# benlaktibyassine/DocQA-MS-Clinical-Document-QA-Assistant-LLM-Microservices-

Measured on AMD Instinct MI355X. Metric: e2e_qa_queries_per_sec, higher is better.
Workload: dtype bf16; 1 GPU; model=llama3-8b generator + minilm-l6 embedder + flat-L2 kNN (k=3), global_batch=256, seq_len=2048, parallelism=dp1, index_vectors=2647, kv_blocks=26451

## Files before the change

### docqa-ms-clinical-document-qa-assistant-llm-microservices-_amd/csrc/bindings.cpp

```cpp
#include <torch/library.h>
#include <algorithm>
#include <tuple>
#include <ATen/ATen.h>
#include <c10/hip/HIPStream.h>
#include <c10/core/DeviceGuard.h>

#include "docqa_kernels.h"

namespace {

hipStream_t stream() { return c10::hip::getCurrentHIPStream().stream(); }

#define CHECK_GPU(t) TORCH_CHECK((t).is_cuda(), #t " must be a GPU tensor")
#define CHECK_BF16(t) TORCH_CHECK((t).scalar_type() == at::kBFloat16, #t " must be bfloat16")
#define CHECK_I32(t) TORCH_CHECK((t).scalar_type() == at::kInt, #t " must be int32")
#define CHECK_CONTIG(t) TORCH_CHECK((t).is_contiguous(), #t " must be contiguous")
#define CHECK_ALIGN16(t) \
  TORCH_CHECK((reinterpret_cast<uintptr_t>((t).data_ptr()) & 15u) == 0, \
              #t " must be 16-byte aligned (storage offset a multiple of 16 bytes)")
static bool kernel_debug() {
  static const bool on = [] {
    const char* e = getenv("DOCQA_KERNEL_DEBUG");
    return e && atoi(e) != 0;
  }();
// ... 579 lines not shown
                                      pml.data_ptr<float>(), order_ptr(order, B), stream()),
           "paged_decode_cascade");
  return out;
}

at::Tensor paged_decode_cascade_grouped(const at::Tensor& q, at::Tensor k_cache, at::Tensor v_cache,
                                        const at::Tensor& block_tables, const at::Tensor& context_lens,
                                        int64_t Hq, double scale, const at::Tensor& prefix_table,
                                        const at::Tensor& prefix_len, int64_t nchunk, const at::Tensor& groups) {
  CHECK_GPU(q); CHECK_BF16(q); CHECK_BF16(k_cache); CHECK_BF16(v_cache);
  CHECK_I32(block_tables); CHECK_I32(context_lens); CHECK_CONTIG(block_tables);
  CHECK_I32(prefix_table); CHECK_I32(prefix_len); CHECK_CONTIG(prefix_table);
  CHECK_I32(groups); CHECK_CONTIG(groups);
  TORCH_CHECK(q.stride(-1) == 1, "q rows must be contiguous");
  const int B = q.size(0);
  const int Hkv = k_cache.size(1), BS = k_cache.size(2), D = k_cache.size(3);
  TORCH_CHECK(D == 128 && BS == 64 && Hq == 4 * Hkv, "grouped decode: head_dim 128, 64-token blocks, GQA 4");
  TORCH_CHECK(block_tables.size(1) <= 256, "grouped decode: block table <= 256 wide (rows <= 64 blocks: the caller)");
  TORCH_CHECK(context_lens.numel() == B && block_tables.size(0) >= B, "grouped decode: B rows");
  TORCH_CHECK(groups.numel() % 4 == 0 && groups.numel() >= 4, "groups: [ngroups, 4]");
  TORCH_CHECK(prefix_table.numel() >= 1 && prefix_len.numel() == 1, "cascade decode: prefix table / length");
  c10::DeviceGuard g(q.device());
  auto out = at::empty({B, Hq * D}, q.options());
  auto f32 = q.options().dtype(at::kFloat);
  auto pacc = at::empty({nchunk, B, Hq, D}, f32);
  auto pml = at::empty({nchunk, B, Hq, 2}, f32);
  CHECK_RC(docqa_paged_decode_cascade_grouped(q.data_ptr(), q.stride(0), k_cache.data_ptr(), v_cache.data_ptr(),
                                              block_tables.data_ptr<int>(), block_tables.size(1),
                                              context_lens.data_ptr<int>(), out.data_ptr(), Hq * D, B, Hq, Hkv,
                                              BS, (float)scale, prefix_table.data_ptr<int>(),
                                              prefix_len.data_ptr<int>(), (int)nchunk, pacc.data_ptr<float>(),
                                              pml.data_ptr<float>(), groups.data_ptr<int>(),
                                              (int)(groups.numel() / 4), stream()),
           "paged_decode_cascade_grouped");
  return out;
}

at::Tensor paged_decode_grouped_fused(const at::Tensor& P, const at::Tensor& positions, const at::Tensor& cos_sin,
                                      const at::Tensor& slot_mapping, at::Tensor k_cache, at::Tensor v_cache,
                                      const at::Tensor& block_tables, const at::Tensor& context_lens, int64_t Hq,
                                      double scale, const at::Tensor& prefix_table, const at::Tensor& prefix_len,
                                      int64_t nchunk, const at::Tensor& plan, const c10::optional<at::Tensor>& tick) {
  CHECK_GPU(P); CHECK_CONTIG(P); CHECK_BF16(k_cache); CHECK_BF16(v_cache);
  CHECK_I32(positions); CHECK_I32(slot_mapping); CHECK_I32(block_tables); CHECK_I32(context_lens);
  CHECK_CONTIG(block_tables); CHECK_I32(prefix_table); CHECK_I32(prefix_len); CHECK_I32(plan); CHECK_CONTIG(plan);
  TORCH_CHECK(P.scalar_type() == at::kFloat && P.dim() == 3, "fused grouped decode: slabs fp32 [S, B, width]");
  TORCH_CHECK(cos_sin.scalar_type() == at::kFloat, "cos_sin must be fp32");
  const int B = P.size(1);
  const int Hkv = k_cache.size(1), BS = k_cache.size(2), D = k_cache.size(3);
  TORCH_CHECK(D == 128 && BS == 64 && Hq == 4 * Hkv && P.size(2) == (Hq + 2 * Hkv) * D,
              "fused grouped decode: head_dim 128, 64-token blocks, GQA 4, packed QKV width");
  TORCH_CHECK(block_tables.size(1) <= 256 && context_lens.numel() == B && block_tables.size(0) >= B &&
              positions.numel() >= B && slot_mapping.numel() >= B, "fused grouped decode: B rows, block table <= 256 wide");
  TORCH_CHECK(plan.dim() == 3 && plan.size(0) == 2 && plan.size(2) == 8, "fused grouped decode: split plan [2, cap, 8]");
  const int cap = plan.size(1);
  c10::DeviceGuard g(P.device());
  auto out = at::empty({B, Hq * D}, P.options().dtype(at::kBFloat16));
  auto f32 = P.options();
  auto ws_acc = at::empty({cap, Hkv, 16, D}, f32);
  auto ws_ml = at::empty({cap, Hkv, 16, 2}, f32);
  int* tick_ptr = nullptr;
  if (tick && tick->defined()) {
    CHECK_GPU((*tick)); CHECK_I32((*tick));
    TORCH_CHECK(tick->numel() >= (int64_t)cap * Hkv, "fused grouped decode: tick needs cap * Hkv entries");
    tick_ptr = tick->data_ptr<int>();
  }
  const int* pp = plan.data_ptr<int>();
  CHECK_RC(docqa_paged_decode_cascade_split(nullptr, 0, k_cache.data_ptr(), v_cache.data_ptr(),
                                            block_tables.data_ptr<int>(), block_tables.size(1),
                                            context_lens.data_ptr<int>(), out.data_ptr(), Hq * D, B, Hq, Hkv, BS,
                                            (float)scale, prefix_table.data_ptr<int>(), prefix_len.data_ptr<int>(),
                                            (int)nchunk, nullptr, nullptr, pp, pp + 8 * cap, cap,
                                            ws_acc.data_ptr<float>(), ws_ml.data_ptr<float>(), 0, stream(), tick_ptr, 1,
                                            P.data_ptr<float>(), P.size(0), positions.data_ptr<int>(),
                                            cos_sin.data_ptr<float>(), slot_mapping.data_ptr<int>()),
           "paged_decode_grouped_fused");
  return out;
}

at::Tensor paged_decode_cascade_split(const at::Tensor& q, at::Tensor k_cache, at::Tensor v_cache,
                                      const at::Tensor& block_tables, const at::Tensor& context_lens,
                                      int64_t Hq, double scale, const at::Tensor& prefix_table,
                                      const at::Tensor& prefix_len, int64_t nchunk, const at::Tensor& plan,
                                      bool defer, const c10::optional<at::Tensor>& tick, bool inline_prefix) {
  CHECK_GPU(q); CHECK_BF16(q);
  TORCH_CHECK(k_cache.dim() == 4, "k_cache: [num_blocks, Hkv, BS, D]");
  const bool f8 = kv_fp8(k_cache, v_cache, k_cache.size(1), k_cache.size(3));
  TORCH_CHECK(!f8 || (inline_prefix && !defer && plan.dim() == 3 && plan.size(0) == 2),
              "split decode (fp8 cache): a [2, cap, 8] plan from block 0 (inline_prefix), not deferred");
  CHECK_I32(block_tables); CHECK_I32(context_lens); CHECK_CONTIG(block_tables);
  CHECK_I32(prefix_table); CHECK_I32(prefix_len); CHECK_CONTIG(prefix_table);
  CHECK_I32(plan); CHECK_CONTIG(plan);
  TORCH_CHECK(q.stride(-1) == 1, "q rows must be contiguous");
  const int B = q.size(0);
  const int Hkv = k_cache.size(1), BS = k_cache.size(2), D = k_cache.size(3);
  TORCH_CHECK(D == 128 && BS == 64 && Hq == 4 * Hkv, "split decode: head_dim 128, 64-token blocks, GQA 4");
  TORCH_CHECK(block_tables.size(1) <= 256, "split decode: block table <= 256 wide (rows <= 64 blocks: the caller)");
  TORCH_CHECK(k_cache.size(0) < (1 << 20), "split decode: < 2^20 KV blocks (packed tile lists)");
  TORCH_CHECK(context_lens.numel() == B && block_tables.size(0) >= B, "split decode: B rows");
  TORCH_CHECK(plan.dim() == 3 && plan.size(0) >= 2 && plan.size(0) <= 3 && plan.size(2) == 8 && plan.size(1) >= 1,
              "plan: [2, cap, 8] (split) or [3, cap, 8] (persistent bins)");
  TORCH_CHECK(prefix_table.numel() >= 1 && prefix_len.numel() == 1, "cascade decode: prefix table / length");
  const int cap = plan.size(1);
  c10::DeviceGuard g(q.device());
  auto out = at::empty({B, Hq * D}, q.options());
  auto f32 = q.options().dtype(at::kFloat);
  auto pacc = f8 ? at::Tensor() : at::empty({nchunk, B, Hq, D}, f32);
  auto pml = f8 ? at::Tensor() : at::empty({nchunk, B, Hq, 2}, f32);
  auto ws_acc = at::empty({cap, Hkv, 16, D}, f32);
  auto ws_ml = at::empty({cap, Hkv, 16, 2}, f32);
  const int* pp = plan.data_ptr<int>();
  int* tick_ptr = nullptr;
  if (tick && tick->defined()) {
    CHECK_GPU((*tick)); CHECK_I32((*tick));
    TORCH_CHECK(tick->numel() >= (int64_t)cap * Hkv, "split decode: tick needs cap * Hkv entries");
    tick_ptr = tick->data_ptr<int>();
  }
  if (f8) {
    TORCH_CHECK(q.dim() == 2 && q.size(1) >= Hq * D && q.stride(0) % 8 == 0, "split decode (fp8 cache): q rows");
    CHECK_ALIGN16(q);
    CHECK_RC(docqa_paged_decode_group_wave8(q.data_ptr(), q.stride(0), k_cache.data_ptr(), v_cache.data_ptr(),
                                            block_tables.data_ptr<int>(), block_tables.size(1),
                                            context_lens.data_ptr<int>(), out.data_ptr(), Hq * D, B, Hq, Hkv, BS,
                                            (float)scale, pp, pp + 8 * cap, cap, ws_acc.data_ptr<float>(),
                                            ws_ml.data_ptr<float>(), stream(), tick_ptr),
             "paged_decode_cascade_split (fp8 cache)");
    return out;
  }
  if (plan.size(0) == 3) {
    CHECK_RC(docqa_paged_decode_cascade_persist(q.data_ptr(), q.stride(0), k_cache.data_ptr(), v_cache.data_ptr(),
                                                block_tables.data_ptr<int>(), block_tables.size(1),
                                                context_lens.data_ptr<int>(), out.data_ptr(), Hq * D, B, Hq, Hkv,
                                                BS, (float)scale, prefix_table.data_ptr<int>(),
                                                prefix_len.data_ptr<int>(), (int)nchunk, pacc.data_ptr<float>(),
                                                pml.data_ptr<float>(), pp, pp + 8 * cap, pp + 16 * cap, cap,
                                                ws_acc.data_ptr<float>(), ws_ml.data_ptr<float>(), stream()),
             "paged_decode_cascade_persist");
    return out;
  }
  CHECK_RC(docqa_paged_decode_cascade_split(q.data_ptr(), q.stride(0), k_cache.data_ptr(), v_cache.data_ptr(),
                                            block_tables.data_ptr<int>(), block_tables.size(1),
                                            context_lens.data_ptr<int>(), out.data_ptr(), Hq * D, B, Hq, Hkv,
                                            BS, (float)scale, prefix_table.data_ptr<int>(),
                                            prefix_len.data_ptr<int>(), (int)nchunk, pacc.data_ptr<float>(),
                                            pml.data_ptr<float>(), pp, pp + 8 * cap, cap, ws_acc.data_ptr<float>(),
                                            ws_ml.data_ptr<float>(), defer ? 1 : 0, stream(), tick_ptr,
                                            inline_prefix ? 1 : 0),
           "paged_decode_cascade_split");
  return out;
}

at::Tensor paged_decode_cascade_rope(at::Tensor qkv, const at::Tensor& positions, const at::Tensor& cos_sin,
                                     const at::Tensor& slot_mapping, at::Tensor k_cache, at::Tensor v_cache,
                                     const at::Tensor& block_tables, const at::Tensor& context_lens,
                                     int64_t Hq, int64_t max_context, double scale,
                                     const at::Tensor& prefix_table, const at::Tensor& prefix_len,
                                     int64_t nchunk, const c10::optional<at::Tensor>& order) {
  CHECK_GPU(qkv); CHECK_BF16(qkv); CHECK_BF16(k_cache); CHECK_BF16(v_cache);
  CHECK_I32(positions); CHECK_I32(slot_mapping); CHECK_I32(block_tables); CHECK_I32(context_lens);
  CHECK_CONTIG(block_tables); CHECK_I32(prefix_table); CHECK_I32(prefix_len); CHECK_CONTIG(prefix_table);
  TORCH_CHECK(qkv.dim() == 2 && qkv.stride(1) == 1, "qkv must be [B, width] with unit stride");
  TORCH_CHECK(cos_sin.scalar_type() == at::kFloat, "cos_sin must be fp32");
  const int B = qkv.size(0);
  const int Hkv = k_cache.size(1), BS = k_cache.size(2), D = k_cache.size(3);
  TORCH_CHECK(D == 128 && BS == 64 && Hq == 4 * Hkv, "cascade decode: head_dim 128, 64-token blocks, GQA 4");
  TORCH_CHECK(qkv.size(1) >= (Hq + 2 * Hkv) * D, "qkv rows narrower than the packed QKV width");
  TORCH_CHECK(positions.numel() == B && slot_mapping.numel() == B && context_lens.numel() == B,
              "positions / slot_mapping / context_lens must have B entries");
  TORCH_CHECK(block_tables.size(1) <= 256, "cascade decode: <= 256 blocks per sequence");
  TORCH_CHECK(prefix_table.numel() >= 1 && prefix_len.numel() == 1, "cascade decode: prefix table / length");
  const int max_parts = docqa_decode_splits(B, Hkv, max_context);
  c10::DeviceGuard g(qkv.device());
  auto out = at::empty({B, Hq * D}, qkv.options());
  auto f32 = qkv.options().dtype(at::kFloat);
  auto tmp_out = at::empty({B, Hq, max_parts, D}, f32);
  auto tmp_ml = at::empty({B, Hq, max_parts, 2}, f32);
  auto pacc = at::empty({nchunk, B, Hq, D}, f32);
  auto pml = at::empty({nchunk, B, Hq, 2}, f32);
  CHECK_RC(docqa_paged_decode_cascade_rope(qkv.data_ptr(), qkv.stride(0), positions.data_ptr<int>(),
                                           cos_sin.data_ptr<float>(), slot_mapping.data_ptr<int>(),
                                           k_cache.data_ptr(), v_cache.data_ptr(), block_tables.data_ptr<int>(),
                                           block_tables.size(1), context_lens.data_ptr<int>(), out.data_ptr(),
                                           Hq * D, tmp_out.data_ptr<float>(), tmp_ml.data_ptr<float>(), B, Hq,
                                           Hkv, BS, max_parts, (float)scale, prefix_table.data_ptr<int>(),
                                           prefix_len.data_ptr<int>(), (int)nchunk, pacc.data_ptr<float>(),
                                           pml.data_ptr<float>(), order_ptr(order, B), stream()),
           "paged_decode_cascade_rope");
  return out;
}

at::Tensor paged_decode_fused(const at::Tensor& P, const at::Tensor& positions, const at::Tensor& cos_sin,
                              const at::Tensor& slot_mapping, at::Tensor k_cache, at::Tensor v_cache,
                              const at::Tensor& block_tables, const at::Tensor& context_lens,
                              int64_t Hq, int64_t max_context, double scale,
                              const c10::optional<at::Tensor>& order, const c10::optional<at::Tensor>& tick) {
  CHECK_GPU(P); CHECK_CONTIG(P); CHECK_BF16(k_cache); CHECK_BF16(v_cache);
  CHECK_I32(positions); CHECK_I32(slot_mapping); CHECK_I32(block_tables); CHECK_I32(context_lens);
  CHECK_CONTIG(block_tables);
  TORCH_CHECK(P.scalar_type() == at::kFloat && P.dim() == 3, "partials must be fp32 [S, B, width]");
  TORCH_CHECK(cos_sin.scalar_type() == at::kFloat, "cos_sin must be fp32");
  const int B = P.size(1);
  const int Hkv = k_cache.size(1), BS = k_cache.size(2), D = k_cache.size(3);
  TORCH_CHECK(D == 128 && P.size(2) == (Hq + 2 * Hkv) * D, "fused decode: head_dim 128, packed QKV width");
  const int max_parts = docqa_decode_splits(B, Hkv, max_context);
  c10::DeviceGuard g(P.device());
  auto out = at::empty({B, Hq * D}, P.options().dtype(at::kBFloat16));
  auto tmp_out = at::empty({B, Hq, max_parts, D}, P.options());
  auto tmp_ml = at::empty({B, Hq, max_parts, 2}, P.options());
  int* tick_ptr = nullptr;
  if (tick && tick->defined()) {
    CHECK_GPU((*tick)); CHECK_I32((*tick));
    TORCH_CHECK(tick->numel() >= (int64_t)B * Hkv, "paged_decode_fused: tick needs B * Hkv entries");
    tick_ptr = tick->data_ptr<int>();
  }
  CHECK_RC(docqa_paged_decode_fused(P.data_ptr<float>(), P.size(0), positions.data_ptr<int>(),
                                    cos_sin.data_ptr<float>(), slot_mapping.data_ptr<int>(),
                                    k_cache.data_ptr(), v_cache.data_ptr(), block_tables.data_ptr<int>(),
                                    block_tables.size(1), context_lens.data_ptr<int>(), out.data_ptr(),
                                    Hq * D, tmp_out.data_ptr<float>(), tmp_ml.data_ptr<float>(), B, Hq,
                                    Hkv, BS, max_parts, (float)scale, order_ptr(order, B), stream(), tick_ptr),
           "paged_decode_fused");
  return out;
}

at::Tensor flash_prefill(const at::Tensor& qkv, const at::Tensor& cu_seqlens, int64_t max_len,
                         int64_t Hq, int64_t Hkv, int64_t D, double scale, bool causal) {
  CHECK_GPU(qkv); CHECK_BF16(qkv); CHECK_I32(cu_seqlens);
  TORCH_CHECK(qkv.stride(-1) == 1 && qkv.size(-1) == (Hq + 2 * Hkv) * D, "qkv layout mismatch");
  const int T = qkv.numel() / qkv.size(-1);
  const int B = cu_seqlens.numel() - 1;
  c10::DeviceGuard g(qkv.device());
  auto out = at::empty({T, Hq * D}, qkv.options());
// ... 908 lines not shown
  m.def("sample(Tensor logits, Tensor inv_temp, Tensor top_k, Tensor top_p, Tensor u) -> Tensor");
  m.def("penalty_window() -> int", &penalty_window);
  m.def("apply_penalties(Tensor(a!) logits, Tensor hist, Tensor hist_n, Tensor last_n, Tensor rep_pen, "
        "Tensor pres_pen, Tensor freq_pen, Tensor? valid=None) -> ()");
  m.def("penalized_argmax(Tensor(a!) logits, int n_valid, Tensor hist, Tensor hist_n, Tensor last_n, "
        "Tensor rep_pen, Tensor pres_pen, Tensor freq_pen, Tensor? valid=None) -> Tensor");
  m.def("top_logprobs_max() -> int", &top_logprobs_max);
  m.def("token_logprobs(Tensor logits, int n_valid, Tensor chosen, Tensor top_n, Tensor(a!) lp, "
        "Tensor(b!) top_ids, Tensor(c!) top_lp) -> ()");
  m.def("decode_advance_hist(Tensor nxt, Tensor(a!) out, Tensor(b!) tokens, Tensor(c!) positions, "
        "Tensor(d!) context_lens, Tensor valid, Tensor(e!) hist, Tensor(f!) hist_n) -> ()");
  m.def("paged_decode(Tensor q, Tensor k_cache, Tensor v_cache, Tensor block_tables, "
        "Tensor context_lens, int Hq, int max_context, float scale, Tensor? order=None) -> Tensor");
  m.def("flash_prefill(Tensor qkv, Tensor cu_seqlens, int max_len, int Hq, int Hkv, int D, "
        "float scale, bool causal) -> Tensor");
  m.def("knn(Tensor xb, Tensor xb_norms, Tensor xq, int k, bool inner_product, int id_offset) "
        "-> (Tensor, Tensor)");
  m.def("pool_l2(Tensor h, Tensor cu_seqlens, bool mean, bool normalize) -> Tensor");
  m.def("coarse_probes(Tensor xq, Tensor cent, Tensor cnorm, int nprobe) -> Tensor");
  m.def("fp32_gemm_nt(Tensor x, Tensor w) -> Tensor");
  m.def("ivfpq_search(Tensor xq, Tensor centroids, Tensor pq, Tensor codes, Tensor ids, "
        "Tensor list_off, Tensor probes, int k) -> (Tensor, Tensor)");
  m.def("ivfpq_search_pt(Tensor xq, Tensor centroids, Tensor pq, Tensor codes, Tensor norms, Tensor ids, "
        "Tensor list_off, Tensor probes, int k, int pc) -> (Tensor, Tensor)");
  m.def("refine_flat(Tensor xb, Tensor xq, Tensor cand, int k, bool ip) -> (Tensor, Tensor)");
  m.def("pq_encode(Tensor x, Tensor centroids, Tensor assign, Tensor pq) -> Tensor");
  m.def("gemm(Tensor a, Tensor w, Tensor? bias, Tensor? residual, int epi) -> Tensor");
  m.def("flash_prefill_paged(Tensor qkv, Tensor cu_seqlens, int max_len, int Hq, int Hkv, int D, "
        "float scale, Tensor k_cache, Tensor v_cache, Tensor block_tables, Tensor ctx_start) -> Tensor");
  m.def("dgemm(Tensor x, Tensor w, int splits) -> Tensor");
  m.def("dgemm_partial(Tensor x, Tensor w, int splits, int tile_rows=64) -> Tensor");
  m.def("embed_rmsnorm(Tensor ids, Tensor table, Tensor w, float eps) -> (Tensor, Tensor)");
  m.def("dgemm_partial_xn(Tensor Pin, Tensor res_in, Tensor(a!) res_out, Tensor gamma, float eps, Tensor w, "
        "int splits) -> Tensor");
  m.def("dgemm_glu_xn(Tensor Pin, Tensor res_in, Tensor(a!) res_out, Tensor gamma, float eps, Tensor w) -> Tensor");
  m.def("gemv(Tensor x, Tensor w, int splits=1, int rows=16, bool glu=False) -> Tensor");
  m.def("gemv_xn(Tensor Pin, Tensor res_in, Tensor(a!) res_out, Tensor gamma, float eps, Tensor w, int splits=1, int rows=16, bool glu=False) -> Tensor");
  m.def("dgemm_add_rmsnorm(Tensor x, Tensor w, int splits, Tensor(a!) residual, Tensor gamma, float eps, "
        "Tensor(t!) tick) -> Tensor");
  m.def("dgemm_glu(Tensor x, Tensor w) -> Tensor");
  m.def("mgemm(Tensor x, Tensor w, int splits, int cfg=0) -> Tensor");
  m.def("mgemm_slab16(Tensor x, Tensor w, int splits, int cfg=0) -> Tensor");
  m.def("mgemm_glu(Tensor x, Tensor w, int cfg=0) -> Tensor");
  m.def("mgemm_tile_n(int cfg) -> int", &mgemm_tile_n);
  m.def("mgemm_argmax(Tensor x, Tensor w, int n_valid, int cfg=0) -> Tensor");
  m.def("dgemm_argmax_val(Tensor x, Tensor w, int n_valid) -> (Tensor, Tensor)");
  m.def("gemv_argmax_val(Tensor x, Tensor w, int n_valid) -> (Tensor, Tensor)");
  m.def("gemv4(Tensor x, Tensor q, Tensor e, int splits=1, int rows=16, int lb=32, int kw=1, bool glu=False) -> Tensor");
  m.def("gemv4_xn(Tensor Pin, Tensor res_in, Tensor(a!) res_out, Tensor gamma, float eps, Tensor q, Tensor e, "
        "int splits=1, int rows=16, int lb=32, int kw=1, bool glu=False) -> Tensor");
  m.def("gemv4_argmax_val(Tensor x, Tensor q, Tensor e, int n_valid, int rows=16, int lb=32, int kw=1) "
        "-> (Tensor, Tensor)");
  m.def("gemv8(Tensor x, Tensor q, Tensor scale, int splits=1, int rows=16, int lb=8, bool glu=False) -> Tensor");
  m.def("gemv8_xn(Tensor Pin, Tensor res_in, Tensor(a!) res_out, Tensor gamma, float eps, Tensor q, Tensor scale, "
        "int splits=1, int rows=16, int lb=8, bool glu=False) -> Tensor");
  m.def("gemv8_argmax_val(Tensor x, Tensor q, Tensor scale, int n_valid, int rows=16, int lb=8) -> (Tensor, Tensor)");
  m.def("dgemm8_partial(Tensor x, Tensor q, Tensor scale, int splits, int tile_rows=64) -> Tensor");
  m.def("dgemm8_glu(Tensor x, Tensor q, Tensor scale) -> Tensor");
  m.def("dgemm8_argmax_val(Tensor x, Tensor q, Tensor scale, int n_valid) -> (Tensor, Tensor)");
  m.def("dgemm8w_partial(Tensor x, Tensor q, Tensor scale, int splits, int tile_rows=128) -> Tensor");
  m.def("dgemm8w_glu(Tensor x, Tensor q, Tensor scale) -> Tensor");
  m.def("dgemm8w_argmax_val(Tensor x, Tensor q, Tensor scale, int n_valid) -> (Tensor, Tensor)");
  m.def("dgemm4_partial(Tensor x, Tensor q, Tensor e, int splits, int tile_rows=64) -> Tensor");
  m.def("dgemm4_glu(Tensor x, Tensor q, Tensor e) -> Tensor");
  m.def("dgemm4_argmax_val(Tensor x, Tensor q, Tensor e, int n_valid) -> (Tensor, Tensor)");
  m.def("pgemm(Tensor x, Tensor w, int epi=0) -> Tensor");
  m.def("pgemm_partial(Tensor x, Tensor w, int splits) -> Tensor");
  m.def("mgemm_argmax_val(Tensor x, Tensor w, int n_valid, int cfg=0) -> (Tensor, Tensor)");
  m.def("pgemm_ok(int M, int N, int K) -> bool", &pgemm_ok);
  m.def("mgemm_ld(Tensor x, Tensor w, int splits, int cfg, bool glu) -> Tensor");
  m.def("group_persist_bins(int cap, int Hkv) -> int", &group_persist_bins);
  m.def("set_decode_trace(Tensor? buf) -> ()", &set_decode_trace);
  m.def("set_group_wave(int on) -> int", &set_group_wave);
  m.def("paged_decode_cascade(Tensor q, Tensor k_cache, Tensor v_cache, Tensor block_tables, "
        "Tensor context_lens, int Hq, int max_context, float scale, Tensor prefix_table, Tensor prefix_len, "
        "int nchunk, Tensor? order=None) -> Tensor");
  m.def("paged_decode_cascade_grouped(Tensor q, Tensor k_cache, Tensor v_cache, Tensor block_tables, "
        "Tensor context_lens, int Hq, float scale, Tensor prefix_table, Tensor prefix_len, int nchunk, "
        "Tensor groups) -> Tensor");
  m.def("kv_copy_rows(Tensor caches, Tensor tab, int num_blocks, int Hkv, int BS, int D) -> ()");
  m.def("kv_copy_rows8(Tensor caches, Tensor tab, int num_blocks, int Hkv, int BS, int D) -> ()");
  m.def("paged_decode_cascade_split(Tensor q, Tensor k_cache, Tensor v_cache, Tensor block_tables, "
        "Tensor context_lens, int Hq, float scale, Tensor prefix_table, Tensor prefix_len, int nchunk, "
        "Tensor plan, bool defer=False, Tensor(t!)? tick=None, bool inline_prefix=False) -> Tensor");
  m.def("paged_decode_grouped_fused(Tensor P, Tensor positions, Tensor cos_sin, Tensor slot_mapping, "
        "Tensor(a!) k_cache, Tensor(b!) v_cache, Tensor block_tables, Tensor context_lens, int Hq, float scale, "
        "Tensor prefix_table, Tensor prefix_len, int nchunk, Tensor plan, Tensor(t!)? tick=None) -> Tensor");
  m.def("paged_decode_cascade_rope(Tensor(a!) qkv, Tensor positions, Tensor cos_sin, Tensor slot_mapping, "
        "Tensor(b!) k_cache, Tensor(c!) v_cache, Tensor block_tables, Tensor context_lens, int Hq, "
        "int max_context, float scale, Tensor prefix_table, Tensor prefix_len, int nchunk, "
        "Tensor? order=None) -> Tensor");
  m.def("paged_decode_fused(Tensor P, Tensor positions, Tensor cos_sin, Tensor slot_mapping, "
        "Tensor(a!) k_cache, Tensor(b!) v_cache, Tensor block_tables, Tensor context_lens, int Hq, "
        "int max_context, float scale, Tensor? order=None, Tensor(t!)? tick=None) -> Tensor");
  m.def("ar_run(Tensor x, bool slabs, Tensor(r!)? residual, Tensor? w, float eps, int rank, int[] regions, "
        "int max_elems, int mode, Tensor(a!) ctr, Tensor(b!) err, int timeout_us=500000) -> Tensor");
  m.def("ar_region_bytes(int max_elems) -> int", &ar_region_bytes);
  m.def("ar_alloc(int bytes) -> int", &ar_alloc);
  m.def("ar_free(int ptr) -> ()", &ar_free);
  m.def("ar_ipc_handle(int ptr) -> Tensor", &ar_ipc_handle);
  m.def("ar_ipc_open(Tensor handle) -> int", &ar_ipc_open);
  m.def("ar_ipc_close(int ptr) -> ()", &ar_ipc_close);
  m.def("add_rmsnorm_splitk(Tensor P, Tensor(a!) residual, Tensor w, float eps) -> Tensor");
  m.def("rope_cache_splitk(Tensor P, Tensor positions, Tensor cos_sin, Tensor? slot_mapping, "
        "Tensor(b!) k_cache, Tensor(c!) v_cache, int Hq, int Hkv, int D) -> Tensor");
}

TORCH_LIBRARY_IMPL(docqa, CUDA, m) {
  m.impl("rmsnorm", &rmsnorm);
  m.impl("add_rmsnorm", &add_rmsnorm);
  m.impl("layernorm", &layernorm);
  m.impl("rope_cache", &rope_cache);
  m.impl("silu_mul", &silu_mul);
  m.impl("silu_mul_splitk", &silu_mul_splitk);
  m.impl("bias_act", &bias_act);
  m.impl("embedding", &embedding);
  m.impl("bert_embed_ln", &bert_embed_ln);
  m.impl("argmax", &argmax);
  m.impl("token_cls_argmax", &token_cls_argmax);
  m.impl("decode_slots", &decode_slots);
  m.impl("decode_advance", &decode_advance);
  m.impl("sample", &sample);
  m.impl("apply_penalties", &apply_penalties);
  m.impl("penalized_argmax", &penalized_argmax);
  m.impl("token_logprobs", &token_logprobs);
  m.impl("decode_advance_hist", &decode_advance_hist);
  m.impl("paged_decode", &paged_decode);
  m.impl("flash_prefill", &flash_prefill);
  m.impl("knn", &knn);
  m.impl("pool_l2", &pool_l2);
  m.impl("ivfpq_search", &ivfpq_search);
  m.impl("ivfpq_search_pt", &ivfpq_search_pt);
  m.impl("refine_flat", &refine_flat);
  m.impl("pq_encode", &pq_encode);
  m.impl("gemm", &gemm);
  m.impl("flash_prefill_paged", &flash_prefill_paged);
  m.impl("dgemm", &dgemm);
  m.impl("dgemm_partial", &dgemm_partial);
  m.impl("embed_rmsnorm", &embed_rmsnorm);
  m.impl("dgemm_partial_xn", &dgemm_partial_xn);
  m.impl("dgemm_glu_xn", &dgemm_glu_xn);
  m.impl("gemv", &gemv);
  m.impl("gemv_xn", &gemv_xn);
  m.impl("dgemm_add_rmsnorm", &dgemm_add_rmsnorm);
  m.impl("dgemm_glu", &dgemm_glu);
  m.impl("mgemm", &mgemm);
  m.impl("mgemm_slab16", &mgemm_slab16);
  m.impl("mgemm_glu", &mgemm_glu);
  m.impl("mgemm_argmax", &mgemm_argmax);
  m.impl("pgemm", &pgemm);
  m.impl("mgemm_ld", &mgemm_ld);
  m.impl("pgemm_partial", &pgemm_partial);
  m.impl("mgemm_argmax_val", &mgemm_argmax_val);
  m.impl("coarse_probes", &coarse_probes);
  m.impl("fp32_gemm_nt", &fp32_gemm_nt);
  m.impl("dgemm_argmax_val", &dgemm_argmax_val);
  m.impl("gemv_argmax_val", &gemv_argmax_val);
  m.impl("gemv4", &gemv4);
  m.impl("gemv4_xn", &gemv4_xn);
  m.impl("gemv4_argmax_val", &gemv4_argmax_val);
  m.impl("gemv8", &gemv8);
  m.impl("gemv8_xn", &gemv8_xn);
  m.impl("gemv8_argmax_val", &gemv8_argmax_val);
  m.impl("dgemm8_partial", &dgemm8_partial);
  m.impl("dgemm8_glu", &dgemm8_glu);
  m.impl("dgemm8_argmax_val", &dgemm8_argmax_val);
  m.impl("dgemm8w_partial", &dgemm8w_partial);
  m.impl("dgemm8w_glu", &dgemm8w_glu);
  m.impl("dgemm8w_argmax_val", &dgemm8w_argmax_val);
  m.impl("dgemm4_partial", &dgemm4_partial);
  m.impl("dgemm4_glu", &dgemm4_glu);
  m.impl("dgemm4_argmax_val", &dgemm4_argmax_val);
  m.impl("paged_decode_fused", &paged_decode_fused);
  m.impl("paged_decode_cascade", &paged_decode_cascade);
  m.impl("paged_decode_cascade_rope", &paged_decode_cascade_rope);
  m.impl("paged_decode_cascade_grouped", &paged_decode_cascade_grouped);
  m.impl("paged_decode_cascade_split", &paged_decode_cascade_split);
  m.impl("paged_decode_grouped_fused", &paged_decode_grouped_fused);
  m.impl("kv_copy_rows", &kv_copy_rows);
  m.impl("kv_copy_rows8", &kv_copy_rows8);
  m.impl("ar_run", &ar_run);
  m.impl("add_rmsnorm_splitk", &add_rmsnorm_splitk);
  m.impl("rope_cache_splitk", &rope_cache_splitk);
}
```

### docqa-ms-clinical-document-qa-assistant-llm-microservices-_amd/csrc/include/docqa_kernels.h

```cpp
#pragma once
#include <hip/hip_runtime.h>
#include <stdint.h>

int docqa_rmsnorm(const void* x, const void* w, void* out, int rows, int H, float eps,
                  hipStream_t s);
int docqa_add_rmsnorm(const void* x, void* residual, const void* w, void* out, int rows, int H,
                      float eps, hipStream_t s);
int docqa_layernorm(const void* x, const void* residual, const void* g, const void* b, void* out,
                    int rows, int H, float eps, hipStream_t s);

int docqa_kv_copy_rows(const uint64_t* caches, int ntensors, const int* tab, int n, int nblocks, int Hkv, int BS,
                       int D, hipStream_t s);
int docqa_rope_cache(void* qkv, const int* positions, const float* cos_sin,
                     const int* slot_mapping, void* k_cache, void* v_cache, int T, int Hq,
                     int Hkv, int D, int row_stride, int BS, hipStream_t s);

int docqa_kv_copy_rows8(const uint64_t* caches, int ntensors, const int* tab, int n, int nblocks, int Hkv, int BS,
                        int D, hipStream_t s);
int docqa_rope_cache8(void* qkv, const int* positions, const float* cos_sin, const int* slot_mapping,
                      void* k_cache, void* v_cache, int T, int Hq, int Hkv, int D, int row_stride, int BS,
                      hipStream_t s);
int docqa_rope_cache_splitk8(const void* P, int slab16, int S, void* qkv_out, const int* positions,
                             const float* cos_sin, const int* slot_mapping, void* k_cache, void* v_cache, int T,
                             int Hq, int Hkv, int D, int row_stride, int BS, hipStream_t s);
int docqa_flash_prefill_paged8(const void* qkv, int row_stride, const int* cu_seqlens, void* out,
                               int o_stride, int B, int max_len, int Hq, int Hkv, int head_dim,
                               float scale, const void* k_cache, const void* v_cache,
                               const int* block_tables, int maxb, const int* ctx_start, int BS,
                               hipStream_t s);
int docqa_paged_decode8(const void* q, int q_stride, const void* k_cache, const void* v_cache,
                        const int* block_tables, int maxb, const int* context_lens, void* out,
                        int out_stride, float* tmp_out, float* tmp_ml, int B, int Hq, int Hkv,
                        int D, int BS, int max_parts, float scale, hipStream_t s);
int docqa_paged_decode_group_wave8(const void* q, int q_stride, const void* k_cache, const void* v_cache,
                                   const int* block_tables, int maxb, const int* context_lens, void* out,
                                   int out_stride, int B, int Hq, int Hkv, int BS, float scale, const int* items,
                                   const int* merges, int cap, float* ws_acc, float* ws_ml, hipStream_t s,
                                   int* tick);

int docqa_silu_mul(const void* gu, void* out, int T, int I, int interleaved, hipStream_t s);
int docqa_silu_mul_splitk16(const void* P, void* out, int S, int T, int I, hipStream_t s);
int docqa_silu_mul_splitk(const float* P, void* out, int S, int T, int I, hipStream_t s);
int docqa_bias_act(const void* x, const void* bias, const void* res, void* out, int T, int N,
                   int gelu, hipStream_t s);

int docqa_embedding(const int* ids, const void* table, void* out, int T, int H, int V, hipStream_t s);
int docqa_decode_slots(const int* block_tables, int maxb, const int* positions, const int* valid,
                       int* slots, int B, int BS, hipStream_t s);
int docqa_decode_advance(const int64_t* nxt, int64_t* out, int* tokens, int* positions,
                         int* context_lens, const int* valid, int B, hipStream_t s);
int docqa_bert_embed_ln(const int* ids, const int* pos, const int* tt, const void* wte,
                        const void* wpe, const void* wtt, const void* g, const void* b, void* out,
                        int T, int H, float eps, hipStream_t s);
int docqa_argmax(const void* logits, int rows, int V, int ld, int is_bf16, float* ws_v, int* ws_i,
                 int splits, int64_t* out, hipStream_t s);
int docqa_token_cls_argmax(const void* h, int ldh, const void* w, const void* bias, int n_rows,
                           int n_valid, int T, int H, int64_t* out, hipStream_t s);
int docqa_sample(const float* logits, int rows, int V, int ld, const float* inv_temp,
                 const int* top_k, const float* top_p, const float* u, int64_t* out,
                 hipStream_t s);

int docqa_penalty_window();
int docqa_apply_penalties(float* logits, int rows, int V, int ld, const int* hist, int W,
                          const int* hist_n, const int* last_n, const float* rep, const float* pres,
                          const float* freq, const int* valid, hipStream_t s);
int docqa_penalized_argmax(void* logits, int rows, int V, int ld, int n_valid, int is_bf16,
                           const int* hist, int W, const int* hist_n, const int* last_n,
                           const float* rep, const float* pres, const float* freq, const int* valid,
                           float* ws_v, int* ws_i, int splits, float* pen_v, int* pen_i,
                           int64_t* out, hipStream_t s);
int docqa_decode_advance_hist(const int64_t* nxt, int64_t* out, int* tokens, int* positions,
                              int* context_lens, const int* valid, int* hist, int W, int* hist_n,
                              int B, hipStream_t s);

int docqa_top_logprobs_max();
int docqa_token_logprobs_splits(int rows, int V, int* chunk_out);
int docqa_token_logprobs(const void* logits, int rows, int n_valid, int ld, int is_bf16, const int64_t* chosen,
                         const int* top_n, float* pm, float* ps, float* ptv, int* pti, float* lp, int* top_ids,
                         float* top_lp, hipStream_t s);

int docqa_paged_decode(const void* q, int q_stride, const void* k_cache, const void* v_cache,
                       const int* block_tables, int maxb, const int* context_lens, void* out,
                       int out_stride, float* tmp_out, float* tmp_ml, int B, int Hq, int Hkv,
                       int D, int BS, int max_parts, float scale, const int* order, hipStream_t s);
int docqa_decode_splits(int B, int Hkv, int max_context);
int docqa_paged_decode_cascade(const void* q, int q_stride, void* k_cache, void* v_cache,
                               const int* block_tables, int maxb, const int* context_lens, void* out,
                               int out_stride, float* tmp_out, float* tmp_ml, int B, int Hq, int Hkv,
                               int BS, int max_parts, float scale, const int* prefix_table,
                               const int* plen, int nchunk, float* pacc, float* pml, const int* order,
                               hipStream_t s);
int docqa_paged_decode_cascade_grouped(const void* q, int q_stride, void* k_cache, void* v_cache,
                                       const int* block_tables, int maxb, const int* context_lens,
                                       void* out, int out_stride, int B, int Hq, int Hkv, int BS,
                                       float scale, const int* prefix_table, const int* plen, int nchunk,
                                       float* pacc, float* pml, const int* groups, int ngroups,
                                       hipStream_t s);
int docqa_paged_decode_cascade_split(const void* q, int q_stride, void* k_cache, void* v_cache,
                                     const int* block_tables, int maxb, const int* context_lens,
                                     void* out, int out_stride, int B, int Hq, int Hkv, int BS,
                                     float scale, const int* prefix_table, const int* plen, int nchunk,
                                     float* pacc, float* pml, const int* items, const int* merges, int cap,
                                     float* ws_acc, float* ws_ml, int defer,
                                     hipStream_t s, int* tick = nullptr, int inline_prefix = 0,
                                     const float* fP = nullptr, int fS = 0, const int* positions = nullptr,
                                     const float* cos_sin = nullptr, const int* slot_mapping = nullptr);
int docqa_paged_decode_cascade_persist(const void* q, int q_stride, void* k_cache, void* v_cache,
                                       const int* block_tables, int maxb, const int* context_lens,
                                       void* out, int out_stride, int B, int Hq, int Hkv, int BS,
                                       float scale, const int* prefix_table, const int* plen, int nchunk,
                                       float* pacc, float* pml, const int* items, const int* merges,
                                       const int* bins, int cap, float* ws_acc, float* ws_ml, hipStream_t s);
int docqa_group_persist_bins(int cap, int Hkv);
int docqa_set_decode_trace(long long* buf);
int docqa_set_group_wave(int on);
int docqa_paged_decode_cascade_rope(void* qkv, int q_stride, const int* positions,
                                    const float* cos_sin, const int* slot_mapping, void* k_cache,
                                    void* v_cache, const int* block_tables, int maxb,
                                    const int* context_lens, void* out, int out_stride,
                                    float* tmp_out, float* tmp_ml, int B, int Hq, int Hkv, int BS,
                                    int max_parts, float scale, const int* prefix_table,
                                    const int* plen, int nchunk, float* pacc, float* pml,
                                    const int* order, hipStream_t s);

int docqa_flash_prefill(const void* qkv, int row_stride, const int* cu_seqlens, void* out,
                        int o_stride, int B, int max_len, int Hq, int Hkv, int head_dim,
                        float scale, int causal, hipStream_t s);

int docqa_flash_prefill_paged(const void* qkv, int row_stride, const int* cu_seqlens, void* out,
                              int o_stride, int B, int max_len, int Hq, int Hkv, int head_dim,
                              float scale, const void* k_cache, const void* v_cache,
                              const int* block_tables, int maxb, const int* ctx_start, int BS,
                              hipStream_t s);

int docqa_dgemm_partial(const void* X, const void* W, float* P, int M, int N, int K, int S,
                        int tile_rows, hipStream_t s);
int docqa_add_rmsnorm_splitk(const float* P, int S, void* residual, const void* w, void* out,
                             int rows, int H, float eps, hipStream_t s);
int docqa_rope_cache_splitk(const float* P, int S, void* qkv_out, const int* positions,
                            const float* cos_sin, const int* slot_mapping, void* k_cache,
                            void* v_cache, int T, int Hq, int Hkv, int D, int row_stride, int BS,
                            hipStream_t s);
int docqa_add_rmsnorm_splitk16(const void* P, int S, void* residual, const void* w, void* out,
                               int rows, int H, float eps, hipStream_t s);
int docqa_rope_cache_splitk16(const void* P, int S, void* qkv_out, const int* positions,
                              const float* cos_sin, const int* slot_mapping, void* k_cache,
                              void* v_cache, int T, int Hq, int Hkv, int D, int row_stride, int BS,
                              hipStream_t s);
size_t docqa_ar_region_bytes(size_t max_elems);
int docqa_ar_alloc(size_t bytes, void** ptr);
int docqa_ar_free(void* ptr);
int docqa_ar_ipc_handle(void* ptr, void* handle_out);
int docqa_ar_ipc_open(const void* handle, void** ptr);
int docqa_ar_ipc_close(void* ptr);
int docqa_ar_run(const void* in, int S, void* out, void* residual, const void* w, float eps, int M, int H,
                 int rank, int nranks, void* const* regions, size_t max_elems, int mode, unsigned* ctr,
                 unsigned* err, long long timeout_us, hipStream_t s);
int docqa_paged_decode_fused(const float* P, int S, const int* positions, const float* cos_sin,
                             const int* slot_mapping, void* k_cache, void* v_cache,
                             const int* block_tables, int maxb, const int* context_lens, void* out,
                             int out_stride, float* tmp_out, float* tmp_ml, int B, int Hq, int Hkv,
                             int BS, int max_parts, float scale, const int* order, hipStream_t s,
                             int* tick = nullptr);
int docqa_dgemm_splits(int N, int K);
int docqa_dgemm_glu(const void* X, const void* W, void* Y, int M, int N, int K, hipStream_t s);
int docqa_dgemm_add_rmsnorm(const void* X, const void* W, float* P, int M, int N, int K, int S, void* residual,
                            const void* gamma, void* out, float eps, int* tick, hipStream_t s);
int docqa_dgemm_partial_xn(const float* Pin, int Sin, const void* res_in, void* res_out, const void* gamma,
                           float eps, const void* W, float* P, int N, int K, int S, hipStream_t s);
int docqa_dgemm_glu_xn(const float* Pin, int Sin, const void* res_in, void* res_out, const void* gamma, float eps,
                       const void* W, void* Y, int N, int K, hipStream_t s);
int docqa_gemv(const void* X, const void* W, void* Y, float* P, int N, int K, int S, int R, int epi,
               const float* Pin, int Sin, const void* res_in, void* res_out, const void* gamma, float eps,
               hipStream_t s);
int docqa_gemv8(const void* X, const void* Wq, const float* scale, void* Y, float* P, int N, int K, int S, int R,
                int LB, int epi, const float* Pin, int Sin, const void* res_in, void* res_out, const void* gamma,
                float eps, hipStream_t s);
int docqa_gemv8_argmax(const void* X, const void* Wq, const float* scale, int64_t* out, float* outv, float* ws_v,
                       int* ws_i, int N, int K, int R, int LB, int n_valid, hipStream_t s);
int docqa_gemv4(const void* X, const void* Wq, const void* E, void* Y, float* P, int N, int K, int S, int R, int LB,
                int KW, int epi, const float* Pin, int Sin, const void* res_in, void* res_out, const void* gamma,
                float eps, hipStream_t s);
int docqa_gemv4_argmax(const void* X, const void* Wq, const void* E, int64_t* out, float* outv, float* ws_v,
                       int* ws_i, int N, int K, int R, int LB, int KW, int n_valid, hipStream_t s);
int docqa_dgemm8_partial(const void* X, const void* Wq, const float* scale, float* P, int M, int N, int K, int S,
                         int tile_rows, hipStream_t s);
int docqa_dgemm8_glu(const void* X, const void* Wq, const float* scale, void* Y, int M, int N, int K, hipStream_t s);
int docqa_dgemm8_argmax(const void* X, const void* Wq, const float* scale, int64_t* out, float* outv, float* ws_v,
                        int* ws_i, int M, int N, int K, int n_valid, hipStream_t s);
// ... 58 lines not shown
```

### docqa-ms-clinical-document-qa-assistant-llm-microservices-_amd/csrc/kernels/attn_decode.hip

```cpp
#include "docqa_common.h"
#include "docqa_asm.h"
#include "docqa_cascade.h"
#include "docqa_norm_row.h"
#include <float.h>
#include <stdlib.h>
#include <type_traits>

using namespace docqa;

constexpr int kMinChunk = 64;
typedef __attribute__((address_space(3))) i16x4 lds_i16x4;

static int hpw_knob() {
  static const int v = [] {
    const char* e = getenv("DOCQA_DECODE_HPW");
    return e ? atoi(e) : 1;
  }();
  return v;
}

static int mfma_nsr() {
  static const int v = [] {
    const char* e = getenv("DOCQA_DECODE_NSR");
    return e ? atoi(e) : 4;
// ... 1131 lines not shown
    const bool mine = (e.y & cbit) != 0;
    const int base = (e.y >> 8) * 64 + ((e.y >> 4) & 1) * TT;
    const uint16_t* kt = ring + (jt % NSR) * 2 * TILE;
    const uint16_t* vt = kt + TILE;
    f32x4 x[2];
#pragma unroll
    for (int c = 0; c < 2; ++c) {
      x[c] = f32x4{0.f, 0.f, 0.f, 0.f};
      const int t = 16 * c + hl;
#pragma unroll
      for (int ks = 0; ks < 4; ++ks) {
        const bf16x8 a = *reinterpret_cast<const bf16x8*>(kt + t * D + (((4 * ks + lg) ^ (t & 15)) << 3));
        x[c] = __builtin_amdgcn_mfma_f32_16x16x32_bf16(a, qf[ks], x[c], 0, 0, 0);
      }
    }
    float mx = -FLT_MAX;
#pragma unroll
    for (int c = 0; c < 2; ++c)
#pragma unroll
      for (int r = 0; r < 4; ++r) {
        const int tok = base + 16 * c + 4 * lg + r;
        const float v = (mine && tok < cL) ? x[c][r] * qs : -FLT_MAX;
        x[c][r] = v;
        mx = fmaxf(mx, v);
      }
    mx = fmaxf(mx, __shfl_xor(mx, 16, 64));
    mx = fmaxf(mx, __shfl_xor(mx, 32, 64));
    const float m_new = fmaxf(m, mx);
    const float alpha = m_new == -FLT_MAX ? 1.f : exp2f(m - m_new);
    float ps = 0.f;
#pragma unroll
    for (int c = 0; c < 2; ++c)
#pragma unroll
      for (int r = 0; r < 4; ++r) {
        const float p = x[c][r] == -FLT_MAX ? 0.f : exp2f(x[c][r] - m_new);
        x[c][r] = p;
        ps += p;
      }
    ps += __shfl_xor(ps, 16, 64);
    ps += __shfl_xor(ps, 32, 64);
    l = l * alpha + ps;
    m = m_new;
#pragma unroll
    for (int dd = 0; dd < 2; ++dd) acc[dd] *= alpha;
#pragma unroll
    for (int c = 0; c < 2; ++c) {
      i16x4 pb;
#pragma unroll
      for (int r = 0; r < 4; ++r) pb[r] = (short)f2bf(x[c][r]);
      const int row = 16 * c + 4 * lg + (hl >> 2), pp = hl & 3;
#pragma unroll
      for (int dd = 0; dd < 2; ++dd) {
        const int ch = 2 * (2 * wave + dd) + (pp >> 1);
        const uint16_t* va = vt + row * D + ((ch ^ vswz(row)) << 3) + 4 * (pp & 1);
        const i16x4 a = __builtin_amdgcn_ds_read_tr16_b64_v4i16((lds_i16x4*)va);
        acc[dd] = __builtin_amdgcn_mfma_f32_16x16x16bf16_1k(a, pb, acc[dd], 0, 0, 0);
      }
    }
  }
  wait_vmcnt<0>();
  if (trace && tid == 0) tr3 = wall_clock64();

  trace_out();
  group_item_finish<SPLIT>(m, l, acc, part, crow, cL, hl, lg, wave, tid, gp, merges, tick, ws_acc, ws_ml, ci,
                           context_lens, B, Hkv, out, out_stride, kvh, P);
}

typedef unsigned int u32x2_t __attribute__((ext_vector_type(2)));
__device__ __forceinline__ float rows4_max(float x) {
  const u32x2_t a = __builtin_amdgcn_permlane16_swap(__float_as_uint(x), __float_as_uint(x), false, false);
  const float h0 = __uint_as_float(a.x), h1 = __uint_as_float(a.y);
  const float y = h0 > h1 ? h0 : h1;
  const u32x2_t b = __builtin_amdgcn_permlane32_swap(__float_as_uint(y), __float_as_uint(y), false, false);
  const float g0 = __uint_as_float(b.x), g1 = __uint_as_float(b.y);
  return g0 > g1 ? g0 : g1;
}
__device__ __forceinline__ float rows4_sum(float x) {
  const u32x2_t a = __builtin_amdgcn_permlane16_swap(__float_as_uint(x), __float_as_uint(x), false, false);
  const float y = __uint_as_float(a.x) + __uint_as_float(a.y);
  const u32x2_t b = __builtin_amdgcn_permlane32_swap(__float_as_uint(y), __float_as_uint(y), false, false);
  return __uint_as_float(b.x) + __uint_as_float(b.y);
}

template <int WAVES, int NSRW>
__global__ __launch_bounds__(64 * WAVES) void paged_decode_group_wave_kernel(
    const uint16_t* __restrict__ q, int q_stride, const uint16_t* __restrict__ k_cache,
    const uint16_t* __restrict__ v_cache, const int* __restrict__ block_tables, int maxb,
    const int* __restrict__ context_lens, int B, int Hkv, float scale,
    uint16_t* __restrict__ out, int out_stride, const int* __restrict__ groups, CascadeIn ci,
    float* __restrict__ ws_acc, float* __restrict__ ws_ml, const int* __restrict__ merges, int* __restrict__ tick) {
  constexpr int G = 4, R = 4, D = 128, TQ = 16, MAXT = kGroupMaxPos * 16;
  constexpr int TILE = TQ * D;
  constexpr int WSLOT = 2 * TILE;
  constexpr int NDT = 8 / WAVES;
  static_assert(WAVES * NSRW * WSLOT * 2 >= WAVES * 8 * 64 * 16 + WAVES * 16 * 2 * 4, "ring reused by the merge");
  __shared__ __attribute__((aligned(16))) uint16_t ring[WAVES * NSRW * WSLOT];
  __shared__ unsigned s_tl[MAXT];
  __shared__ int s_nt;

  const int kvh = blockIdx.x, grp = blockIdx.y;
  const int tid = threadIdx.x, lane = tid & 63;
  const int wave = __builtin_amdgcn_readfirstlane(tid >> 6);
  const int hl = lane & 15, lg = lane >> 4;
  long long* trace = g_group_trace;
  long long tr0 = 0, tr1 = 0, tr2 = 0, tr3 = 0;
  if (trace && tid == 0) tr0 = wall_clock64();
  const int P = ci.plen ? *ci.plen : 0;
  const int* gp = groups + 8 * grp;
  int rows[R], Ls[R];
#pragma unroll
  for (int r = 0; r < R; ++r) {
    const int row = gp[r];
    rows[r] = row >= 0 && row < B ? row : -1;
    Ls[r] = rows[r] >= 0 ? context_lens[rows[r]] : 0;
  }
  if (rows[0] < 0 && rows[1] < 0 && rows[2] < 0 && rows[3] < 0) return;
  const int lo = gp[4], hi = min(gp[5], maxb), part = gp[6];

  if (wave == 0) {
    const int pos = max(P >> 6, lo) + lane;
    int ids[R], nq[R], mk[R];
#pragma unroll
    for (int r = 0; r < R; ++r) ids[r] = rows[r] >= 0 && pos < hi ? block_tables[(size_t)rows[r] * maxb + pos] : -1;
    bool alive[R];
#pragma unroll
    for (int r = 0; r < R; ++r) {
      alive[r] = pos < hi && 64 * pos < Ls[r];
      ids[r] = alive[r] ? ids[r] : -1;
    }
    int cnt = 0;
#pragma unroll
    for (int r = 0; r < R; ++r) {
      bool first = alive[r];
#pragma unroll
      for (int r2 = 0; r2 < r; ++r2) first = first && !(alive[r2] && ids[r2] == ids[r]);
      int mask = 0, need = 0;
      if (first) {
#pragma unroll
        for (int r2 = 0; r2 < R; ++r2)
          if (alive[r2] && ids[r2] == ids[r]) {
            mask |= 1 << r2;
            need = max(need, min(4, (Ls[r2] - 64 * pos + TQ - 1) / TQ));
          }
      }
      nq[r] = need;
      mk[r] = mask;
      cnt += need;
    }
    int off = cnt;
#pragma unroll
    for (int o = 1; o < 64; o <<= 1) {
      const int v = __shfl_up(off, o, 64);
      if (lane >= o) off += v;
    }
    const int total = __shfl(off, 63, 64);
    off -= cnt;
#pragma unroll
    for (int r = 0; r < R; ++r)
      for (int h = 0; h < nq[r]; ++h) s_tl[off++] = ((unsigned)ids[r] << 12) | (pos << 6) | (h << 4) | mk[r];
    if (lane == 0) s_nt = total;
  }
  const int crow = rows[hl >> 2], cL = Ls[hl >> 2], cbit = 1 << (hl >> 2);
  bf16x8 qf[4];
  {
    const uint16_t* qp = q + (size_t)max(crow, 0) * q_stride + (size_t)(kvh * G + (hl & 3)) * D + lg * 8;
#pragma unroll
    for (int ks = 0; ks < 4; ++ks) {
      const uint4 v = crow >= 0 ? *reinterpret_cast<const uint4*>(qp + ks * 32) : make_uint4(0, 0, 0, 0);
      qf[ks] = __builtin_bit_cast(bf16x8, v);
    }
  }
  __syncthreads();
  const int nt = s_nt;
  if (trace && tid == 0) tr1 = wall_clock64();

  const float qs = scale * kLog2e;
  const uint32_t wbase = lds_u32(ring) + (uint32_t)(wave * NSRW * WSLOT * 2);
  const int prow = lane >> 4, pslot = lane & 15;
  const int mine_nt = nt > wave ? (nt - wave + WAVES - 1) / WAVES : 0;
  auto stage = [&](int i) {
    const unsigned e = s_tl[wave + WAVES * i];
    const size_t row0 = ((size_t)(e >> 12) * Hkv + kvh) * 64 + ((e >> 4) & 3) * TQ;
    const uint16_t* kp = k_cache + row0 * D;
    const uint16_t* vp = v_cache + row0 * D;
    const uint32_t dst = wbase + (uint32_t)((i % NSRW) * WSLOT * 2);
#pragma unroll
    for (int c = 0; c < 4; ++c) {
      const int t = 4 * c + prow;
      glds16<true>(kp + t * D + ((pslot ^ t) << 3), dst + c * 1024);
      glds16<true>(vp + t * D + ((pslot ^ vswz(t)) << 3), dst + TILE * 2 + c * 1024);
    }
  };
#pragma unroll
  for (int i = 0; i < NSRW - 1; ++i)
    if (i < mine_nt) stage(i);
  float m = -FLT_MAX, l = 0.f;
  f32x4 o8[8];
#pragma unroll
  for (int dt = 0; dt < 8; ++dt) o8[dt] = f32x4{0.f, 0.f, 0.f, 0.f};
  for (int i = 0; i < mine_nt; ++i) {
    if (i + NSRW - 1 < mine_nt) {
      stage(i + NSRW - 1);
      wait_vmcnt<8 * (NSRW - 1)>();
    } else {
      wait_vmcnt<0>();
    }
    if (trace && tid == 0 && i == 0) tr2 = wall_clock64();
    const unsigned e = s_tl[wave + WAVES * i];
    const bool mine = (e & cbit) != 0;
    const int base = ((e >> 6) & 63) * 64 + ((e >> 4) & 3) * TQ;
    const uint16_t* kt = ring + (wave * NSRW + i % NSRW) * WSLOT;
    const uint16_t* vt = kt + TILE;
    f32x4 x = f32x4{0.f, 0.f, 0.f, 0.f};
#pragma unroll
    for (int ks = 0; ks < 4; ++ks) {
      const bf16x8 a = *reinterpret_cast<const bf16x8*>(kt + hl * D + (((4 * ks + lg) ^ hl) << 3));
      x = __builtin_amdgcn_mfma_f32_16x16x32_bf16(a, qf[ks], x, 0, 0, 0);
    }
    float mx = -FLT_MAX;
#pragma unroll
    for (int r = 0; r < 4; ++r) {
      const int tok = base + 4 * lg + r;
      const float v = (mine && tok < cL) ? x[r] * qs : -FLT_MAX;
      x[r] = v;
      mx = fmaxf(mx, v);
    }
    mx = rows4_max(mx);
    const float m_new = fmaxf(m, mx);
    const float alpha = m_new == -FLT_MAX ? 1.f : __builtin_amdgcn_exp2f(m - m_new);
    float ps = 0.f;
#pragma unroll
    for (int r = 0; r < 4; ++r) {
      const float p = x[r] == -FLT_MAX ? 0.f : __builtin_amdgcn_exp2f(x[r] - m_new);
      x[r] = p;
      ps += p;
    }
    ps = rows4_sum(ps);
    l = l * alpha + ps;
    m = m_new;
    i16x4 pb;
#pragma unroll
    for (int r = 0; r < 4; ++r) pb[r] = (short)f2bf(x[r]);
    const int row = 4 * lg + (hl >> 2), pp = hl & 3;
#pragma unroll
    for (int dt = 0; dt < 8; ++dt) {
      o8[dt] *= alpha;
      const int ch = 2 * dt + (pp >> 1);
      const uint16_t* va = vt + row * D + ((ch ^ vswz(row)) << 3) + 4 * (pp & 1);
      const i16x4 a = __builtin_amdgcn_ds_read_tr16_b64_v4i16((lds_i16x4*)va);
      o8[dt] = __builtin_amdgcn_mfma_f32_16x16x16bf16_1k(a, pb, o8[dt], 0, 0, 0);
    }
  }
  if (trace && tid == 0) tr3 = wall_clock64();

  __syncthreads();
  f32x4* s_o = reinterpret_cast<f32x4*>(ring);
  float* s_ml = reinterpret_cast<float*>(ring) + WAVES * 8 * 64 * 4;
#pragma unroll
  for (int dt = 0; dt < 8; ++dt) s_o[(wave * 8 + dt) * 64 + lane] = o8[dt];
  if (lg == 0) {
    s_ml[(wave * 16 + hl) * 2] = m;
    s_ml[(wave * 16 + hl) * 2 + 1] = l;
  }
  __syncthreads();
  float mw[WAVES], lw[WAVES], M = -FLT_MAX;
#pragma unroll
  for (int u = 0; u < WAVES; ++u) {
    mw[u] = s_ml[(u * 16 + hl) * 2];
    lw[u] = s_ml[(u * 16 + hl) * 2 + 1];
    M = fmaxf(M, mw[u]);
  }
  f32x4 acc[NDT];
#pragma unroll
  for (int dd = 0; dd < NDT; ++dd) acc[dd] = f32x4{0.f, 0.f, 0.f, 0.f};
  float L = 0.f;
#pragma unroll
  for (int u = 0; u < WAVES; ++u) {
    const float f = mw[u] == -FLT_MAX ? 0.f : exp2f(mw[u] - M);
    L += f * lw[u];
#pragma unroll
    for (int dd = 0; dd < NDT; ++dd) acc[dd] += f * s_o[(u * 8 + NDT * wave + dd) * 64 + lane];
  }
  if (trace && tid == 0) {
    long long* t = trace + ((size_t)blockIdx.y * gridDim.x + blockIdx.x) * 8;
    t[0] = tr0; t[1] = tr1; t[2] = tr2; t[3] = tr3; t[4] = wall_clock64(); t[5] = nt;
    t[6] = __builtin_amdgcn_s_getreg((31 << 11) | 4);
    t[7] = __builtin_amdgcn_s_getreg(20 | (3 << 11)) & 15;
  }
  group_item_finish<true, NDT>(M, L, acc, part, crow, cL, hl, lg, wave, tid, gp, merges, tick, ws_acc, ws_ml, ci,
                          context_lens, B, Hkv, out, out_stride, kvh, P);
}

__device__ __forceinline__ i16x4 widen4_fp8(uint32_t c) {
  const bf16x2 a = __builtin_amdgcn_cvt_scalef32_pk_bf16_fp8(c, 1.0f, false);
  const bf16x2 b = __builtin_amdgcn_cvt_scalef32_pk_bf16_fp8(c, 1.0f, true);
  const uint2 u{__builtin_bit_cast(uint32_t, a), __builtin_bit_cast(uint32_t, b)};
  return __builtin_bit_cast(i16x4, u);
}

template <int NSRW>
__global__ __launch_bounds__(256) void paged_decode_group_wave8_kernel(
    const uint16_t* __restrict__ q, int q_stride, const uint8_t* __restrict__ k_cache,
    const uint8_t* __restrict__ v_cache, const int* __restrict__ block_tables, int maxb,
    const int* __restrict__ context_lens, int B, int Hkv, float scale,
    uint16_t* __restrict__ out, int out_stride, const int* __restrict__ groups, CascadeIn ci,
    float* __restrict__ ws_acc, float* __restrict__ ws_ml, const int* __restrict__ merges, int* __restrict__ tick) {
  constexpr int WAVES = 4, G = 4, R = 4, D = 128, TQ = 16, MAXT = kGroupMaxPos * 16;
  constexpr int TILE = TQ * D;
  constexpr int WSLOT = 2 * TILE;
  constexpr int NDT = 8 / WAVES;
  static_assert(WAVES * NSRW * WSLOT >= WAVES * 8 * 64 * 16 + WAVES * 16 * 2 * 4, "ring reused by the merge");
  __shared__ __attribute__((aligned(16))) uint8_t ring[WAVES * NSRW * WSLOT];
  __shared__ unsigned s_tl[MAXT];
  __shared__ int s_nt;

  const int kvh = blockIdx.x, grp = blockIdx.y;
  const int tid = threadIdx.x, lane = tid & 63;
  const int wave = __builtin_amdgcn_readfirstlane(tid >> 6);
  const int hl = lane & 15, lg = lane >> 4;
  const int P = ci.plen ? *ci.plen : 0;
  const int* gp = groups + 8 * grp;
  int rows[R], Ls[R];
#pragma unroll
  for (int r = 0; r < R; ++r) {
    const int row = gp[r];
    rows[r] = row >= 0 && row < B ? row : -1;
    Ls[r] = rows[r] >= 0 ? context_lens[rows[r]] : 0;
  }
  if (rows[0] < 0 && rows[1] < 0 && rows[2] < 0 && rows[3] < 0) return;
  const int lo = gp[4], hi = min(gp[5], maxb), part = gp[6];

  if (wave == 0) {
    const int pos = max(P >> 6, lo) + lane;
    int ids[R], nq[R], mk[R];
#pragma unroll
    for (int r = 0; r < R; ++r) ids[r] = rows[r] >= 0 && pos < hi ? block_tables[(size_t)rows[r] * maxb + pos] : -1;
    bool alive[R];
#pragma unroll
    for (int r = 0; r < R; ++r) {
      alive[r] = pos < hi && 64 * pos < Ls[r];
      ids[r] = alive[r] ? ids[r] : -1;
    }
    int cnt = 0;
#pragma unroll
    for (int r = 0; r < R; ++r) {
      bool first = alive[r];
#pragma unroll
      for (int r2 = 0; r2 < r; ++r2) first = first && !(alive[r2] && ids[r2] == ids[r]);
      int mask = 0, need = 0;
      if (first) {
#pragma unroll
        for (int r2 = 0; r2 < R; ++r2)
          if (alive[r2] && ids[r2] == ids[r]) {
            mask |= 1 << r2;
            need = max(need, min(4, (Ls[r2] - 64 * pos + TQ - 1) / TQ));
          }
      }
      nq[r] = need;
      mk[r] = mask;
      cnt += need;
    }
    int off = cnt;
#pragma unroll
    for (int o = 1; o < 64; o <<= 1) {
      const int v = __shfl_up(off, o, 64);
      if (lane >= o) off += v;
    }
    const int total = __shfl(off, 63, 64);
    off -= cnt;
#pragma unroll
    for (int r = 0; r < R; ++r)
      for (int h = 0; h < nq[r]; ++h) s_tl[off++] = ((unsigned)ids[r] << 12) | (pos << 6) | (h << 4) | mk[r];
    if (lane == 0) s_nt = total;
  }
  const int crow = rows[hl >> 2], cL = Ls[hl >> 2], cbit = 1 << (hl >> 2);
  bf16x8 qf[4];
  {
    const uint16_t* qp = q + (size_t)max(crow, 0) * q_stride + (size_t)(kvh * G + (hl & 3)) * D + lg * 8;
#pragma unroll
    for (int ks = 0; ks < 4; ++ks) {
      const uint4 v = crow >= 0 ? *reinterpret_cast<const uint4*>(qp + ks * 32) : make_uint4(0, 0, 0, 0);
      qf[ks] = __builtin_bit_cast(bf16x8, v);
    }
  }
  __syncthreads();
  const int nt = s_nt;

  const float qs = scale * kLog2e;
  const uint32_t wbase = lds_u32(ring) + (uint32_t)(wave * NSRW * WSLOT);
  const int prow = lane >> 3, pslot = lane & 7;
  const int mine_nt = nt > wave ? (nt - wave + WAVES - 1) / WAVES : 0;
  auto stage = [&](int i) {
    const unsigned e = s_tl[wave + WAVES * i];
    const size_t row0 = ((size_t)(e >> 12) * Hkv + kvh) * 64 + ((e >> 4) & 3) * TQ;
    const uint8_t* kp = k_cache + row0 * D;
    const uint8_t* vp = v_cache + row0 * D;
    const uint32_t dst = wbase + (uint32_t)((i % NSRW) * WSLOT);
#pragma unroll
    for (int c = 0; c < 2; ++c) {
      const int t = 8 * c + prow;
      glds16<true>(kp + t * D + ((pslot ^ ((t >> 1) & 7)) << 4), dst + c * 1024);
      glds16<true>(vp + (t ^ ((t >> 2) & 1)) * D + (pslot << 4), dst + TILE + c * 1024);
    }
  };
#pragma unroll
  for (int i = 0; i < NSRW - 1; ++i)
    if (i < mine_nt) stage(i);
  float m = -FLT_MAX, l = 0.f;
  f32x4 o8[8];
#pragma unroll
  for (int dt = 0; dt < 8; ++dt) o8[dt] = f32x4{0.f, 0.f, 0.f, 0.f};
  for (int i = 0; i < mine_nt; ++i) {
    if (i + NSRW - 1 < mine_nt) {
      stage(i + NSRW - 1);
      wait_vmcnt<4 * (NSRW - 1)>();
    } else {
      wait_vmcnt<0>();
    }
    const unsigned e = s_tl[wave + WAVES * i];
    const bool mine = (e & cbit) != 0;
    const int base = ((e >> 6) & 63) * 64 + ((e >> 4) & 3) * TQ;
    const uint8_t* kt = ring + (wave * NSRW + i % NSRW) * WSLOT;
    const uint8_t* vt = kt + TILE;
    f32x4 x = f32x4{0.f, 0.f, 0.f, 0.f};
#pragma unroll
    for (int ks = 0; ks < 4; ++ks) {
      const uint2 c = *reinterpret_cast<const uint2*>(kt + hl * D + (((2 * ks + (lg >> 1)) ^ ((hl >> 1) & 7)) << 4) +
                                                      (lg & 1) * 8);
      const bf16x8 a = __builtin_bit_cast(bf16x8, widen8_fp8(c));
      x = __builtin_amdgcn_mfma_f32_16x16x32_bf16(a, qf[ks], x, 0, 0, 0);
    }
    float mx = -FLT_MAX;
#pragma unroll
    for (int r = 0; r < 4; ++r) {
      const int tok = base + 4 * lg + r;
      const float v = (mine && tok < cL) ? x[r] * qs : -FLT_MAX;
      x[r] = v;
      mx = fmaxf(mx, v);
    }
    mx = rows4_max(mx);
    const float m_new = fmaxf(m, mx);
    const float alpha = m_new == -FLT_MAX ? 1.f : __builtin_amdgcn_exp2f(m - m_new);
    float ps = 0.f;
#pragma unroll
    for (int r = 0; r < 4; ++r) {
      const float p = x[r] == -FLT_MAX ? 0.f : __builtin_amdgcn_exp2f(x[r] - m_new);
      x[r] = p;
      ps += p;
    }
    ps = rows4_sum(ps);
    l = l * alpha + ps;
    m = m_new;
    i16x4 pb;
#pragma unroll
    for (int r = 0; r < 4; ++r) pb[r] = (short)f2bf(x[r]);
    uint2 w[4];
#pragma unroll
    for (int j = 0; j < 4; ++j) {
      const int t = 4 * lg + j;
      w[j] = *reinterpret_cast<const uint2*>(vt + (t ^ ((t >> 2) & 1)) * D + hl * 8);
    }
#pragma unroll
    for (int ih = 0; ih < 2; ++ih) {
      const uint32_t w0 = ih ? w[0].y : w[0].x, w1 = ih ? w[1].y : w[1].x;
      const uint32_t w2 = ih ? w[2].y : w[2].x, w3 = ih ? w[3].y : w[3].x;
      const uint32_t a01 = __builtin_amdgcn_perm(w1, w0, 0x05010400u), a23 = __builtin_amdgcn_perm(w3, w2, 0x05010400u);
      const uint32_t c01 = __builtin_amdgcn_perm(w1, w0, 0x07030602u), c23 = __builtin_amdgcn_perm(w3, w2, 0x07030602u);
      const uint32_t tr[4] = {__builtin_amdgcn_perm(a23, a01, 0x05040100u), __builtin_amdgcn_perm(a23, a01, 0x07060302u),
                              __builtin_amdgcn_perm(c23, c01, 0x05040100u), __builtin_amdgcn_perm(c23, c01, 0x07060302u)};
// ... 424 lines not shown
  const CascadeIn ci{pacc, pml, plen, nchunk, nullptr};
  static const int nsr = [] {
    const char* e = getenv("DOCQA_GROUP_NSR");
    return e && atoi(e) == 4 ? 4 : 3;
  }();
  if (nsr == 4)
    paged_decode_group_kernel<4><<<dim3(Hkv, ngroups), 256, 0, s>>>(
        (const uint16_t*)q, q_stride, (const uint16_t*)k_cache, (const uint16_t*)v_cache, block_tables, maxb,
        context_lens, B, Hkv, scale, (uint16_t*)out, out_stride, groups, ci);
  else
    paged_decode_group_kernel<3><<<dim3(Hkv, ngroups), 256, 0, s>>>(
        (const uint16_t*)q, q_stride, (const uint16_t*)k_cache, (const uint16_t*)v_cache, block_tables, maxb,
        context_lens, B, Hkv, scale, (uint16_t*)out, out_stride, groups, ci);
  DOCQA_CHECK_LAUNCH();
  return 0;
}

static int cascade_prefix_forked(const void* q, int q_stride, int B, int Hq, int Hkv, float scale, void* k_cache,
                                 void* v_cache, const int* prefix_table, const int* plen, int BS, int nchunk,
                                 float* pacc, float* pml, hipStream_t s, hipEvent_t* join) {
  static const bool fork = [] {
    const char* e = getenv("DOCQA_CASCADE_FORK");
    return !(e && atoi(e) == 0);
  }();
  *join = nullptr;
  hipStream_t side = s;
  hipEvent_t ev_fork = nullptr, ev_join = nullptr;
  if (fork) {
    static hipStream_t streams[64] = {};
    static hipEvent_t evs[64][2] = {};
    int dev = 0;
    if (hipGetDevice(&dev) == hipSuccess && dev >= 0 && dev < 64) {
      hipStreamCaptureStatus cs = hipStreamCaptureStatusNone;
      if (!streams[dev] && hipStreamIsCapturing(s, &cs) == hipSuccess && cs == hipStreamCaptureStatusNone) {
        if (hipStreamCreateWithFlags(&streams[dev], hipStreamNonBlocking) != hipSuccess ||
            hipEventCreateWithFlags(&evs[dev][0], hipEventDisableTiming) != hipSuccess ||
            hipEventCreateWithFlags(&evs[dev][1], hipEventDisableTiming) != hipSuccess)
          streams[dev] = nullptr;
      }
      if (streams[dev] && evs[dev][0] && evs[dev][1]) {
        side = streams[dev];
        ev_fork = evs[dev][0];
        ev_join = evs[dev][1];
      }
    }
  }
  if (side != s) {
    if (hipEventRecord(ev_fork, s) != hipSuccess || hipStreamWaitEvent(side, ev_fork, 0) != hipSuccess) return -3;
  }
  const int rc = docqa_cascade_prefix(q, q_stride, B, Hq, Hkv, scale, k_cache, v_cache, prefix_table, plen, BS,
                                      nchunk, pacc, pml, nullptr, nullptr, side);
  if (rc) return rc;
  if (side != s) {
    if (hipEventRecord(ev_join, side) != hipSuccess) return -3;
    *join = ev_join;
  }
  return 0;
}

static int g_group_wave = -1;
static bool group_wave_on() {
  if (g_group_wave < 0) {
    const char* e = getenv("DOCQA_GROUP_WAVE");
    const int v = e ? atoi(e) : 1;
    g_group_wave = v >= 0 && v <= 4 ? v : 0;
  }
  return g_group_wave > 0;
}

int docqa_set_group_wave(int v) {
  group_wave_on();
  const int was = g_group_wave;
  if (v >= 0) g_group_wave = v <= 4 ? v : 0;
  return was;
}

int docqa_paged_decode_cascade_split(const void* q, int q_stride, void* k_cache, void* v_cache,
                                     const int* block_tables, int maxb, const int* context_lens,
                                     void* out, int out_stride, int B, int Hq, int Hkv, int BS,
                                     float scale, const int* prefix_table, const int* plen, int nchunk,
                                     float* pacc, float* pml, const int* items, const int* merges, int cap,
                                     float* ws_acc, float* ws_ml, int defer, hipStream_t s, int* tick,
                                     int inline_prefix, const float* fP, int fS, const int* positions,
                                     const float* cos_sin, const int* slot_mapping) {
  if (B == 0) return 0;
  if (BS != 64 || maxb > kGroupMaxTable || Hq != 4 * Hkv || nchunk < 1 || nchunk > kCascadeMaxChunks || cap < 1)
    return -1;
  if (inline_prefix && defer) return -1;
  hipEvent_t ev_join = nullptr;
  if (!inline_prefix) {
    const int rc = defer ? cascade_prefix_forked(q, q_stride, B, Hq, Hkv, scale, k_cache, v_cache, prefix_table,
                                                 plen, BS, nchunk, pacc, pml, s, &ev_join)
                         : docqa_cascade_prefix(q, q_stride, B, Hq, Hkv, scale, k_cache, v_cache, prefix_table, plen,
                                                BS, nchunk, pacc, pml, nullptr, nullptr, s);
    if (rc) return rc;
  }
  const CascadeIn ci{pacc, pml, inline_prefix ? nullptr : plen, nchunk, nullptr};
  static const int nsr = [] {
    const char* e = getenv("DOCQA_GROUP_NSR");
    return e && atoi(e) == 4 ? 4 : 3;
  }();
  int* tk = (tick && !defer) ? tick : nullptr;
  if (fP) {
    if (!inline_prefix || defer || fS < 1 || !positions || !cos_sin || !slot_mapping) return -1;
    const FusedQKV fz{fP, fS, positions, cos_sin, slot_mapping, Hq};
    paged_decode_group_kernel<3, true, true><<<dim3(Hkv, cap), 256, 0, s>>>(
        nullptr, 0, (const uint16_t*)k_cache, (const uint16_t*)v_cache, block_tables, maxb, context_lens, B, Hkv,
        scale, (uint16_t*)out, out_stride, items, ci, ws_acc, ws_ml, merges, tk, fz);
    DOCQA_CHECK_LAUNCH();
    if (tk) return 0;
  } else if (group_wave_on()) {
#define DOCQA_WAVE_LAUNCH(W_, N_)                                                                                 \
  paged_decode_group_wave_kernel<W_, N_><<<dim3(Hkv, cap), 64 * W_, 0, s>>>(                                     \
      (const uint16_t*)q, q_stride, (const uint16_t*)k_cache, (const uint16_t*)v_cache, block_tables, maxb,       \
      context_lens, B, Hkv, scale, (uint16_t*)out, out_stride, items, ci, ws_acc, ws_ml, merges, tk)
    switch (g_group_wave) {
      case 2: DOCQA_WAVE_LAUNCH(2, 3); break;
      case 3: DOCQA_WAVE_LAUNCH(2, 4); break;
      case 4: DOCQA_WAVE_LAUNCH(1, 4); break;
      default: DOCQA_WAVE_LAUNCH(4, 2); break;
    }
#undef DOCQA_WAVE_LAUNCH
  } else if (nsr == 4)
    paged_decode_group_kernel<4, true><<<dim3(Hkv, cap), 256, 0, s>>>(
        (const uint16_t*)q, q_stride, (const uint16_t*)k_cache, (const uint16_t*)v_cache, block_tables, maxb,
        context_lens, B, Hkv, scale, (uint16_t*)out, out_stride, items, ci, ws_acc, ws_ml, merges, tk);
  else
    paged_decode_group_kernel<3, true><<<dim3(Hkv, cap), 256, 0, s>>>(
        (const uint16_t*)q, q_stride, (const uint16_t*)k_cache, (const uint16_t*)v_cache, block_tables, maxb,
        context_lens, B, Hkv, scale, (uint16_t*)out, out_stride, items, ci, ws_acc, ws_ml, merges, tk);
  DOCQA_CHECK_LAUNCH();
  if (tk) return 0;
  if (ev_join && hipStreamWaitEvent(s, ev_join, 0) != hipSuccess) return -3;
  group_split_merge_kernel<<<dim3(Hkv, defer ? cap : (cap + 1) / 2), 256, 0, s>>>(merges, ws_acc, ws_ml, context_lens, B, Hkv,
                                                          (uint16_t*)out, out_stride, ci);
  DOCQA_CHECK_LAUNCH();
  return 0;
}

int docqa_paged_decode_group_wave8(const void* q, int q_stride, const void* k_cache, const void* v_cache,
                                   const int* block_tables, int maxb, const int* context_lens, void* out,
                                   int out_stride, int B, int Hq, int Hkv, int BS, float scale, const int* items,
                                   const int* merges, int cap, float* ws_acc, float* ws_ml, hipStream_t s,
                                   int* tick) {
  if (B == 0) return 0;
  if (BS != 64 || maxb > kGroupMaxTable || Hq != 4 * Hkv || cap < 1) return -1;
  const CascadeIn ci{nullptr, nullptr, nullptr, 1, nullptr};
  paged_decode_group_wave8_kernel<4><<<dim3(Hkv, cap), 256, 0, s>>>(
      (const uint16_t*)q, q_stride, (const uint8_t*)k_cache, (const uint8_t*)v_cache, block_tables, maxb,
      context_lens, B, Hkv, scale, (uint16_t*)out, out_stride, items, ci, ws_acc, ws_ml, merges, tick);
  DOCQA_CHECK_LAUNCH();
  if (tick) return 0;
  group_split_merge_kernel<<<dim3(Hkv, (cap + 1) / 2), 256, 0, s>>>(merges, ws_acc, ws_ml, context_lens, B, Hkv,
                                                                   (uint16_t*)out, out_stride, ci);
  DOCQA_CHECK_LAUNCH();
  return 0;
}

int docqa_paged_decode_cascade_persist(const void* q, int q_stride, void* k_cache, void* v_cache,
                                       const int* block_tables, int maxb, const int* context_lens,
                                       void* out, int out_stride, int B, int Hq, int Hkv, int BS,
                                       float scale, const int* prefix_table, const int* plen, int nchunk,
                                       float* pacc, float* pml, const int* items, const int* merges,
                                       const int* bins, int cap, float* ws_acc, float* ws_ml, hipStream_t s) {
  if (B == 0) return 0;
  if (BS != 64 || maxb > kGroupMaxTable || Hq != 4 * Hkv || nchunk < 1 || nchunk > kCascadeMaxChunks || cap < 1)
    return -1;
  hipEvent_t ev_join = nullptr;
  const int rc = cascade_prefix_forked(q, q_stride, B, Hq, Hkv, scale, k_cache, v_cache, prefix_table, plen, BS,
                                       nchunk, pacc, pml, s, &ev_join);
  if (rc) return rc;
  const CascadeIn ci{pacc, pml, plen, nchunk, nullptr};
  const int nb = group_persist_bins(cap, Hkv);
  paged_decode_group_persist_kernel<3><<<dim3(Hkv, nb), 256, 0, s>>>(
      (const uint16_t*)q, q_stride, (const uint16_t*)k_cache, (const uint16_t*)v_cache, block_tables, maxb,
      context_lens, B, Hkv, scale, items, bins, ci, ws_acc, ws_ml);
  DOCQA_CHECK_LAUNCH();
  if (ev_join && hipStreamWaitEvent(s, ev_join, 0) != hipSuccess) return -3;
  group_split_merge_kernel<<<dim3(Hkv, cap), 256, 0, s>>>(merges, ws_acc, ws_ml, context_lens, B, Hkv,
                                                          (uint16_t*)out, out_stride, ci);
  DOCQA_CHECK_LAUNCH();
  return 0;
}

int docqa_group_persist_bins(int cap, int Hkv) { return group_persist_bins(cap, Hkv); }

int docqa_set_decode_trace(long long* buf) {
  return hipMemcpyToSymbol(HIP_SYMBOL(g_group_trace), &buf, sizeof(buf)) == hipSuccess ? 0 : -1;
}

template <int D>
__global__ __launch_bounds__(D) void paged_decode_reduce(const float* __restrict__ tmp_out,
                                                         const float* __restrict__ tmp_ml,
                                                         const int* __restrict__ context_lens,
                                                         uint16_t* __restrict__ out,
                                                         int out_stride, int Hq, int max_parts,
                                                         CascadeIn ci = CascadeIn{}) {
  const int h = blockIdx.x, b = blockIdx.y, d = threadIdx.x;
  const int P = ci.plen ? *ci.plen : 0;
  const int L = context_lens[b] - P;
  if (L <= 0) {
    out[(size_t)b * out_stride + (size_t)h * D + d] = 0;
    return;
  }
  const int chunk = split_chunk(L, max_parts);
  const int np = min(max_parts, (L + chunk - 1) / chunk);
  const int nc = ci.plen ? cascade_parts(P, ci.nchunk) : 0;
  const size_t base = ((size_t)b * Hq + h) * max_parts;
  const size_t B = gridDim.y;
  float M = -FLT_MAX;
  for (int p = 0; p < np; ++p) M = fmaxf(M, tmp_ml[(base + p) * 2]);
  for (int c = 0; c < nc; ++c) M = fmaxf(M, ci.ml[((c * B + b) * Hq + h) * 2]);
  float num = 0.f, den = 0.f;
  for (int p = 0; p < np; ++p) {
    const float w = exp2f(tmp_ml[(base + p) * 2] - M);
    num += w * tmp_out[(base + p) * D + d];
    den += w * tmp_ml[(base + p) * 2 + 1];
  }
  for (int c = 0; c < nc; ++c) {
    const size_t r = (c * B + b) * Hq + h;
    const float pm = ci.ml[r * 2];
    const float w = (pm == -FLT_MAX) ? 0.f : exp2f(pm - M);
    num += w * ci.acc[r * D + d];
    den += w * ci.ml[r * 2 + 1];
  }
  out[(size_t)b * out_stride + (size_t)h * D + d] = f2bf(den > 0.f ? num / den : 0.f);
}

int docqa_paged_decode(const void* q, int q_stride, const void* k_cache, const void* v_cache,
                       const int* block_tables, int maxb, const int* context_lens, void* out,
                       int out_stride, float* tmp_out, float* tmp_ml, int B, int Hq, int Hkv,
                       int D, int BS, int max_parts, float scale, const int* order, hipStream_t s) {
  if (B == 0) return 0;
  if (D != 128 || (BS & (BS - 1)) != 0 || Hq % Hkv != 0) return -1;
  CascadeIn oi{};
  oi.order = order;
  int log2BS = 0;
  while ((1 << log2BS) < BS) ++log2BS;
  const int G = Hq / Hkv;
  dim3 grid(Hkv, B, max_parts);
  const bool direct = max_parts == 1;
  static const int u_env = [] {
    const char* e = getenv("DOCQA_DECODE_U");
    return e ? atoi(e) : 0;
  }();
#define DEC_K(GG, UU, DIR)                                                                    \
  paged_decode_kernel<GG, 128, UU, DIR><<<grid, 256, 0, s>>>(                                 \
      (const uint16_t*)q, q_stride, (const uint16_t*)k_cache, (const uint16_t*)v_cache,       \
      block_tables, maxb, context_lens, tmp_out, tmp_ml, Hkv, BS, log2BS, max_parts, scale,   \
      (uint16_t*)out, out_stride)
#define DEC(GG, UU)                                                                           \
  do {                                                                                        \
    if (direct) DEC_K(GG, UU, true);                                                          \
    else DEC_K(GG, UU, false);                                                                \
  } while (0)
  if (mfma_decode_on(G) && BS == 64 && maxb <= 256 && (G == 4 || G == 8)) {
#define DMFMA(GG)                                                                             \
    do {                                                                                      \
      if (direct && Hkv % 2 == 0 && hpw_knob() == 2)                                          \
        paged_decode_mfma_kernel<GG, true, 2><<<dim3(Hkv / 2, B, 1), 256, 0, s>>>(            \
            (const uint16_t*)q, q_stride, (const uint16_t*)k_cache, (const uint16_t*)v_cache, \
            block_tables, maxb, context_lens, tmp_out, tmp_ml, Hkv, max_parts, scale,         \
            (uint16_t*)out, out_stride, oi);                                         \
      else if (direct)                                                                        \
        paged_decode_mfma_kernel<GG, true><<<grid, 256, 0, s>>>(                              \
            (const uint16_t*)q, q_stride, (const uint16_t*)k_cache, (const uint16_t*)v_cache, \
            block_tables, maxb, context_lens, tmp_out, tmp_ml, Hkv, max_parts, scale,         \
            (uint16_t*)out, out_stride, oi);                                         \
// ... 274 lines not shown
```

### docqa-ms-clinical-document-qa-assistant-llm-microservices-_amd/engine/llm_engine.py

```python
from __future__ import annotations

import json
import itertools
import os
import time
from dataclasses import dataclass, field

import numpy as np
import torch

from .. import ops
from ..parallel import comm
from ..utils import tracing
from ..models.llama import AttnMeta, LlamaModel
from .kv_cache import KVCache, TailCache, chain_keys, resolve_kv_dtype

_PREFILL_LOG = os.environ.get("DOCQA_PREFILL_LOG") == "1"
_PREFILL_DUMP = os.environ.get("DOCQA_PREFILL_DUMP", "")
_DECODE_DUMP = os.environ.get("DOCQA_DECODE_DUMP", "")
_DECODE_DUMP_SKIP = [int(os.environ.get("DOCQA_DECODE_DUMP_SKIP", "1"))]


@dataclass
class SamplingParams:
# ... 53 lines not shown
    @property
    def done_event(self):
        return self.events[2] if self.events else None

    @property
    def start_event(self):
        return self.events[0] if self.events else None


@dataclass
class GenStats:
    prefill_s: float = 0.0
    decode_s: float = 0.0
    prompt_tokens: int = 0
    generated_tokens: int = 0
    cached_tokens: int = 0
    attn_kv_blocks: int = 0
    attn_batches: int = 0


def _bucket(n: int, cap: int) -> int:
    b = 1
    while b < n:
        b *= 2
    return min(b, cap)


def _prefill_inputs(prompts: list[list[int]], tables: list[list[int]], cached: list[int], BS: int):
    new = np.array([len(p) - c for p, c in zip(prompts, cached)], dtype=np.int64)
    total = int(new.sum())
    ids = np.fromiter(itertools.chain.from_iterable(p[c:] for p, c in zip(prompts, cached)),
                      dtype=np.int32, count=total)
    cu = np.zeros(len(prompts) + 1, dtype=np.int32)
    np.cumsum(new, out=cu[1:])
    rows = np.repeat(np.arange(len(prompts)), new)
    pos = np.arange(total, dtype=np.int64) - cu[:-1].astype(np.int64)[rows] + np.asarray(cached, np.int64)[rows]
    tbm = np.zeros((len(tables), max(len(t) for t in tables)), dtype=np.int64)
    for r, t in enumerate(tables):
        tbm[r, :len(t)] = t
    slots = tbm[rows, pos // BS] * BS + pos % BS
    return ids, pos.astype(np.int32), slots.astype(np.int32), cu


def ring_of(stream: list[int], W: int) -> tuple[torch.Tensor, int]:
    n = len(stream)
    row = torch.zeros(W, dtype=torch.int32)
    m = min(n, W)
    if m:
        idx = torch.arange(n - m, n) % W
        row[idx] = torch.tensor(stream[n - m:], dtype=torch.int32)
    return row, n


def logprob_entry(lp: float, top_ids: list[int], top_lp: list[float]) -> tuple:
    n = top_ids.index(-1) if -1 in top_ids else len(top_ids)
    return float(lp), [(int(i), float(v)) for i, v in zip(top_ids[:n], top_lp[:n])]


def _upload(dst: torch.Tensor, src: torch.Tensor) -> None:
    if dst.device.type == "cuda":
        dst.copy_(src.pin_memory(), non_blocking=True)
    else:
        dst.copy_(src)


_GROUP_NOPREFIX = os.environ.get("DOCQA_GROUP_NOPREFIX", "1") == "1"
_GROUP_NOPREFIX_MIN = int(os.environ.get("DOCQA_GROUP_NOPREFIX_MIN_BATCH", "32"))


def _split_groups_on() -> bool:
    return os.environ.get("DOCQA_GROUP_SPLIT", "1") == "1"


def _persist_groups_on() -> bool:
    return _split_groups_on() and os.environ.get("DOCQA_GROUP_PERSIST", "0") == "1"


def _inline_prefix_on() -> bool:
    return _split_groups_on() and os.environ.get("DOCQA_GROUP_INLINE_PREFIX", "1") == "1"


def _group_wave_on() -> bool:
    return os.environ.get("DOCQA_GROUP_WAVE", "1") != "0"


def _defer_groups_on() -> bool:
    return _split_groups_on() and os.environ.get("DOCQA_GROUP_DEFER", "0") == "1"


def _identity_groups(bp: int, dev, hkv: int = 8) -> torch.Tensor:
    cap = (bp + 1) // 2
    if _split_groups_on():
        persist = _persist_groups_on()
        all_partial = persist or _defer_groups_on()
        rows = max(bp, 1) * max(1, int(os.environ.get("DOCQA_GROUP_CAP_MULT", "1")))
        g = torch.full((3 if persist else 2, rows, 8), -1, dtype=torch.int32)
        g[:2, :, 4:] = 0
        g[0, :, 6] = -1
        nq = (bp + 3) // 4
        for i in range(nq):
            q = list(range(4 * i, min(4 * i + 4, bp)))
            g[0, i, :len(q)] = torch.tensor(q, dtype=torch.int32)
            g[0, i, 5] = 1 << 20
            if all_partial:
                g[0, i, 4] = 0
                g[0, i, 6] = i
                g[0, i, 7] = i
                g[1, i, :len(q)] = torch.tensor(q, dtype=torch.int32)
                g[1, i, 4], g[1, i, 5] = i, 1
            else:
                g[0, i, 6] = -1
        if persist:
            nb = ops.persist_bins(max(bp, 1), hkv)
            for i in range(nq):
                g[2, i % nb, i // nb] = i
        return g.to(dev)
    g = torch.full((cap * 4,), -1, dtype=torch.int32)
    g[:bp] = torch.arange(bp, dtype=torch.int32)
    return g.to(dev)


class _DecodeGraph:

    def __init__(self, eng: "LLMEngine", bp: int):
        dev = eng.device
        self.bp = bp
        self.tokens = torch.zeros(bp, dtype=torch.int32, device=dev)
        self.positions = torch.zeros(bp, dtype=torch.int32, device=dev)
        self.context_lens = torch.zeros(bp, dtype=torch.int32, device=dev)
        self.valid = torch.zeros(bp, dtype=torch.int32, device=dev)
        self.block_tables = torch.zeros(bp, eng.max_blocks_per_seq, dtype=torch.int32, device=dev)
        self.inv_temp = torch.ones(bp, dtype=torch.float32, device=dev)
        self.top_k = torch.zeros(bp, dtype=torch.int32, device=dev)
        self.top_p = torch.ones(bp, dtype=torch.float32, device=dev)
        self.out = torch.zeros(bp, dtype=torch.long, device=dev)
        self.hist = torch.zeros(bp, ops.PENALTY_WINDOW, dtype=torch.int32, device=dev)
        self.hist_n = torch.zeros(bp, dtype=torch.int32, device=dev)
        self.last_n = torch.zeros(bp, dtype=torch.int32, device=dev)
        self.rep_pen = torch.ones(bp, dtype=torch.float32, device=dev)
        self.pres_pen = torch.zeros(bp, dtype=torch.float32, device=dev)
        self.freq_pen = torch.zeros(bp, dtype=torch.float32, device=dev)
        self.penalized = False
        self.lp_n = torch.full((bp,), -1, dtype=torch.int32, device=dev)
        self.lp = torch.zeros(bp, dtype=torch.float32, device=dev)
        self.lp_top_ids = torch.full((bp, ops.TOP_LOGPROBS_MAX), -1, dtype=torch.int32, device=dev)
        self.lp_top = torch.full((bp, ops.TOP_LOGPROBS_MAX), float("-inf"), dtype=torch.float32, device=dev)
        self.logprobs = False
        self.shared_table = torch.zeros(eng.max_blocks_per_seq, dtype=torch.int32, device=dev)
        self.shared_len = torch.zeros(1, dtype=torch.int32, device=dev)
        self.order = torch.arange(bp, dtype=torch.int32, device=dev)
        self.order_key = None
        self.groups = _identity_groups(bp, dev, eng.model.hkv)
        self.groups_key = None
        self.cascade = False
        self.greedy = True
        self.graph = None
        self.hkv = eng.model.hkv
        self.groups_fit = eng.max_blocks_per_seq <= ops.GROUP_MAX_BLOCKS

    @classmethod
    def view_of(cls, master: "_DecodeGraph", bp: int) -> "_DecodeGraph":
        g = cls.__new__(cls)
        g.bp = bp
        for name in ("tokens", "positions", "context_lens", "valid", "block_tables", "inv_temp",
                     "top_k", "top_p", "out", "hist", "hist_n", "last_n", "rep_pen", "pres_pen", "freq_pen",
                     "lp_n", "lp", "lp_top_ids", "lp_top"):
            setattr(g, name, getattr(master, name)[:bp])
        g.shared_table, g.shared_len = master.shared_table, master.shared_len
        g.order = torch.arange(bp, dtype=torch.int32, device=master.tokens.device)
        g.order_key = None
        g.groups = _identity_groups(bp, master.tokens.device, master.hkv)
        g.groups_key = None
        g.cascade, g.greedy, g.graph = False, True, None
        g.penalized = False
        g.logprobs = False
        g.groups_fit = master.groups_fit
        g.hkv = master.hkv
        return g


class LLMEngine:
    def __init__(self, model: LlamaModel, max_batch: int = 64, max_context: int = 2048,
                 block_size: int = 64, num_blocks: int | None = None, use_graphs: bool = True,
                 max_prefill_tokens: int = 65536, prefix_cache: bool = True,
                 kv_mem_fraction: float | None = None, kv_dtype: str | None = None):
        self.model = model
        self.cfg = model.cfg
        self.device = model.device
        self.kv_dtype = resolve_kv_dtype(kv_dtype, model.dtype)
        self.kv_fp8 = self.kv_dtype == ops.KV_FP8
        if (self.kv_fp8 and self.device.type == "cuda"
                and not ops.kv_fp8_shape_ok(model.hq, model.hkv, model.cfg.head_dim, block_size)):
            raise ValueError("FP8 KV cache on the GPU: head_dim 128, block_size 64 and 4 or 8 query heads per "
                             f"KV head (got head_dim {model.cfg.head_dim}, block_size {block_size}, "
                             f"{model.hq} / {model.hkv} heads)")
        self.max_batch = max_batch
        self.block_size = block_size
        self.max_blocks_per_seq = (max_context + block_size - 1) // block_size
        self.max_context = self.max_blocks_per_seq * block_size
        sw = getattr(model.cfg, "sliding_window", None)
        if sw is not None and self.max_context > sw:
            raise ValueError(f"max_context {self.max_context} exceeds the model's sliding window {sw}: "
                             "the attention kernels attend to the whole context")
        if getattr(model, "tp", 1) > 1:
            from ..parallel import comm
            car = comm.custom_all_reduce()
            if car is not None:
                cap = car.max_elems // model.cfg.hidden // block_size * block_size
                max_prefill_tokens = max(block_size, min(max_prefill_tokens, cap))
        self.max_prefill_tokens = max_prefill_tokens
        if num_blocks is None:
            num_blocks = max_batch * self.max_blocks_per_seq + 1
            if kv_mem_fraction is None and os.environ.get("DOCQA_KV_MEM_FRACTION"):
                kv_mem_fraction = float(os.environ["DOCQA_KV_MEM_FRACTION"])
            if kv_mem_fraction and self.device.type == "cuda":
                fb = self._blocks_from_free_memory(model, block_size, kv_mem_fraction)
                if num_blocks <= self._blocks_from_free_memory(model, block_size, 0.95):
                    num_blocks = max(num_blocks, fb)
                elif fb >= self.max_blocks_per_seq + 1:
                    num_blocks = fb
                else:
                    raise MemoryError(f"KV pool: {fb} blocks fit in {kv_mem_fraction:.2f} of the free HBM, "
                                      f"one {self.max_context}-token sequence needs {self.max_blocks_per_seq + 1}")
        num_blocks = self._agree_across_tp(model, num_blocks)
        self.kv = KVCache(self.cfg.layers, num_blocks, model.hkv, self.cfg.head_dim, block_size,
                          self.device, self.kv_dtype)
        self.use_graphs = use_graphs and self.device.type == "cuda"
        self.tune_decode_gemms = os.environ.get("DOCQA_TUNE_DECODE", "0") == "1"
        self.prefix_cache = prefix_cache and os.environ.get("DOCQA_PREFIX_CACHE", "1") == "1"
        self.cascade = os.environ.get("DOCQA_CASCADE", "1") == "1"
        self.cascade_min_tokens = int(os.environ.get("DOCQA_CASCADE_MIN_TOKENS", "128"))
        self.cascade_min_batch = int(os.environ.get("DOCQA_CASCADE_MIN_BATCH", "4"))
        self.lpt = os.environ.get("DOCQA_DECODE_LPT", "1") == "1"
        self.group_decode = os.environ.get("DOCQA_DECODE_GROUP", "1") == "1"
        self._use_pc = self.prefix_cache and hasattr(self.kv.allocator, "match_alloc_batch")
        cap = min(int(os.environ.get("DOCQA_TAIL_CACHE", "4096")), num_blocks // 8)
        self.tail = TailCache(self.kv.allocator, block_size, cap) if self._use_pc and cap > 0 else None
        self._graphs: dict[tuple, _DecodeGraph] = {}
        self._pool = None
        self.stats = GenStats()

    @staticmethod
    def _agree_across_tp(model, num_blocks: int) -> int:
        import torch.distributed as dist

        from ..parallel import comm

        st = comm.state()
        if getattr(model, "tp", 1) > 1 and st.tp_size > 1 and dist.is_initialized():
            t = torch.tensor([num_blocks], dtype=torch.int64)
            dist.all_reduce(t, op=dist.ReduceOp.MIN, group=st.tp_cpu_group or st.tp_group)
            num_blocks = int(t.item())
        return num_blocks

    def _blocks_from_free_memory(self, model, block_size: int, fraction: float) -> int:
        cfg = model.cfg
        free, _ = torch.cuda.mem_get_info(self.device)
        el = torch.finfo(model.dtype).bits // 8
        block_bytes = KVCache.bytes_per_block(cfg.layers, model.hkv, cfg.head_dim, block_size, self.kv_dtype)
        per_tok = (6 * cfg.hidden + (model.hq + 2 * model.hkv) * cfg.head_dim + 3 * model.inter) * el
        headroom = 2 * self.max_prefill_tokens * per_tok + (6 << 30)
        budget = int(free * fraction) - headroom
        return max(0, budget // block_bytes)

    def _prefill(self, prompts: list[list[int]], tables: list[list[int]],
                 cached: list[int] | None = None, greedy: bool = False) -> torch.Tensor:
        dev, BS = self.device, self.block_size
        cached = list(cached or [0] * len(prompts))
        budget = max(BS, self.max_prefill_tokens // BS * BS)
        for k, (p, tb) in enumerate(zip(prompts, tables)):
            while len(p) - cached[k] > budget:
                end = cached[k] + budget
                self._prefill([p[:end]], [tb], [cached[k]])
                cached[k] = end
        firsts = []
        i = 0
        while i < len(prompts):
            j, tok = i, 0
            while j < len(prompts) and (j == i or tok + len(prompts[j]) - cached[j] <= self.max_prefill_tokens):
                tok += len(prompts[j]) - cached[j]
                j += 1
            ids, pos, slots, cu = _prefill_inputs(prompts[i:j], tables[i:j], cached[i:j], BS)
            t_ids = torch.from_numpy(ids).to(dev, non_blocking=True)
            meta = AttnMeta(
                prefill=True,
                positions=torch.from_numpy(pos).to(dev, non_blocking=True),
                slot_mapping=torch.from_numpy(slots).to(dev, non_blocking=True),
                cu_seqlens=torch.from_numpy(cu).to(dev, non_blocking=True),
                max_len=max(len(p) - c for p, c in zip(prompts[i:j], cached[i:j])))
            if any(cached[i:j]):
                maxb = max(len(tb) for tb in tables[i:j])
                bt = torch.zeros(j - i, maxb, dtype=torch.int32)
                for r, tb in enumerate(tables[i:j]):
                    bt[r, :len(tb)] = torch.tensor(tb, dtype=torch.int32)
                meta.block_tables = bt.to(dev, non_blocking=True)
                meta.prefix_lens = torch.tensor(cached[i:j], dtype=torch.int32).to(dev, non_blocking=True)
            last = torch.from_numpy(cu[1:].astype(np.int64) - 1).to(dev, non_blocking=True)
            if _PREFILL_DUMP and meta.block_tables is not None:
                os.makedirs(_PREFILL_DUMP, exist_ok=True)
                torch.save({"cu": torch.tensor(cu, dtype=torch.int32), "ctx": torch.tensor(cached[i:j], dtype=torch.int32),
                            "bt": meta.block_tables.cpu()},
                           os.path.join(_PREFILL_DUMP, f"prefill_{time.time_ns()}.pt"))
            if _PREFILL_LOG:
                new = [len(p) - c for p, c in zip(prompts[i:j], cached[i:j])]
                print(json.dumps({"prefill_chunk": j - i, "new_sum": sum(new), "new_max": max(new),
                                  "cached_mean": sum(cached[i:j]) / (j - i), "cached_max": max(cached[i:j]),
                                  "cached_min": min(cached[i:j])}), flush=True)
            firsts.append(self.model.forward(t_ids, meta, self.kv.caches, logits_index=last, greedy_ids=greedy))
            i = j
        return torch.cat(firsts, 0)

    def _step_body(self, g: _DecodeGraph) -> None:
        meta = self._decode_meta(g)
        if g.logprobs:
            nxt = self._pick_logprobs(self.model.forward(g.tokens, meta, self.kv.caches), g)
            if g.penalized:
                ops.decode_advance_hist(nxt.long().contiguous(), g.out, g.tokens, g.positions, g.context_lens,
                                        g.valid, g.hist, g.hist_n)
            else:
                ops.decode_advance(nxt.long().contiguous(), g.out, g.tokens, g.positions, g.context_lens, g.valid)
            return
        if g.penalized:
            logits = self.model.forward(g.tokens, meta, self.kv.caches)
            if g.greedy:
                nxt = self._penalized_greedy(logits, g)
            else:
                nxt = self._select(logits, g)
            ops.decode_advance_hist(nxt.long().contiguous(), g.out, g.tokens, g.positions, g.context_lens,
                                    g.valid, g.hist, g.hist_n)
            return
        if g.greedy:
            nxt = self.model.forward(g.tokens, meta, self.kv.caches, greedy_ids=True)
        else:
            nxt = self._select(self.model.forward(g.tokens, meta, self.kv.caches), g)
        ops.decode_advance(nxt.long().contiguous(), g.out, g.tokens, g.positions, g.context_lens, g.valid)

    def _decode_meta(self, g: _DecodeGraph) -> AttnMeta:
        slots = ops.decode_slots(g.block_tables, g.positions, g.valid, self.block_size)
        meta = AttnMeta(prefill=False, positions=g.positions, slot_mapping=slots,
                        block_tables=g.block_tables, context_lens=g.context_lens,
                        max_context=self.max_context, seq_order=g.order if self.lpt else None)
        if g.cascade:
            meta.shared_table, meta.shared_len = g.shared_table, g.shared_len
            meta.cascade_chunks = self._cascade_chunks(g.bp)
            if self.group_decode and g.groups_fit and ops.grouped_decode_ok(
                    self.kv.caches[0][0], g.block_tables, self.model.hq, max_blocks=ops.GROUP_MAX_BLOCKS):
                meta.decode_groups = g.groups
                meta.decode_defer = g.groups.dim() == 3 and _defer_groups_on()
                meta.decode_inline = (g.groups.dim() == 3 and g.groups.shape[0] == 2 and _inline_prefix_on()
                                      and not _defer_groups_on())
            if self.kv_fp8 and self.device.type == "cuda" and not meta.decode_inline:
                meta.shared_table = meta.shared_len = meta.decode_groups = None
        return meta

    def _select(self, logits, g: _DecodeGraph, full=None):
        from .. import ops

        if g.greedy:
            return self.model.greedy(logits)
        src = self.model.full_logits(logits) if full is None else full
        full = src.float()
        if g.penalized:
            if not full.is_contiguous() or full.data_ptr() in (logits.data_ptr(), src.data_ptr()):
                full = full.clone(memory_format=torch.contiguous_format)
            R = full.shape[0]
            ops.apply_penalties(full, g.hist[:R], g.hist_n[:R], g.last_n[:R], g.rep_pen[:R], g.pres_pen[:R],
                                g.freq_pen[:R], g.valid[:R])
        u = torch.rand(full.shape[0], device=full.device)
        return ops.sample(full, g.inv_temp, g.top_k, g.top_p, u)

    def _penalized_greedy(self, logits, g: _DecodeGraph, full=None):
        full = self.model.full_logits(logits) if full is None else full
        R = full.shape[0]
        return ops.penalized_argmax(full, full.shape[1], g.hist[:R], g.hist_n[:R], g.last_n[:R], g.rep_pen[:R],
                                    g.pres_pen[:R], g.freq_pen[:R], g.valid[:R])

    def _pick_logprobs(self, logits, g: _DecodeGraph):
        full = self.model.full_logits(logits)
        if g.penalized and g.greedy:
            nxt = self._penalized_greedy(logits, g, full=full.clone())
        elif g.greedy:
            nxt = self.model.greedy(logits)
        else:
            nxt = self._select(logits, g, full=full)
        R = full.shape[0]
        ops.token_logprobs(full, self.cfg.vocab_size, nxt.long().contiguous(), g.lp_n[:R], g.lp[:R],
                           g.lp_top_ids[:R], g.lp_top[:R])
        return nxt

    def _get_graph(self, bp: int, greedy: bool, cascade: bool = False, fit: bool = True,
                   penalized: bool = False, logprobs: bool = False) -> _DecodeGraph:
        fit = fit or self.max_blocks_per_seq <= ops.GROUP_MAX_BLOCKS
        key = (bp, greedy, cascade, fit, penalized, logprobs)
        g = self._graphs.get(key)
        if g is None:
            g = _DecodeGraph(self, bp)
            g.greedy = greedy
            g.penalized = penalized
            g.logprobs = logprobs
            g.cascade = cascade
            g.groups_fit = fit
            self._graphs[key] = g
        return g

    def groups_fit(self, end_lens: list[int]) -> bool:
        if self.max_blocks_per_seq <= ops.GROUP_MAX_BLOCKS:
            return True
        BS = self.block_size
        return all((n + BS - 1) // BS <= ops.GROUP_MAX_BLOCKS for n in end_lens)

    def set_order(self, g: _DecodeGraph, lens: list[int], key=None) -> None:
        if key is not None and g.order_key == key:
            return
        order = sorted(range(len(lens)), key=lambda i: -lens[i]) + list(range(len(lens), g.bp))
        _upload(g.order, torch.tensor(order, dtype=torch.int32))
        g.order_key = key

    def set_groups(self, g: _DecodeGraph, tables: list[list[int]], lens: list[int], skip: int,
                   key=None, ids: list | None = None) -> None:
        if not self.group_decode or (key is not None and g.groups_key == key):
            return
        skip_in = skip
        if (ids is not None and g.groups.dim() == 3 and getattr(g, "plan_ids", None) is not None
                and g.plan_skip == skip_in and len(ids) * 4 >= len(g.plan_ids) * 3):
            plan = ops.remap_plan_rows(g.plan_host, g.plan_ids, ids)
            if plan is not None:
                _upload(g.groups, plan)
                g.groups_key = key
                return
        if g.groups.dim() == 3:
            cap = g.groups.shape[1]
            quads = ops.pack_decode_groups(tables, lens, skip, self.block_size, (g.bp + 1) // 2)
            if _inline_prefix_on() and not _defer_groups_on() and g.groups.shape[0] == 2:
                skip = 0
            bins = ops.persist_bins(cap, self.model.hkv) if g.groups.shape[0] == 3 else 0

# ... 423 lines not shown
```

### docqa-ms-clinical-document-qa-assistant-llm-microservices-_amd/models/llama.py

```python
from __future__ import annotations

import math
import os
import zlib
from dataclasses import dataclass, field
from typing import NamedTuple

import torch
import torch.nn.functional as F

from .. import ops
from ..parallel import comm

_CASCADE_ROPE = os.environ.get("DOCQA_CASCADE_ROPE", "0") == "1"
_PREFILL_TRIM = os.environ.get("DOCQA_PREFILL_TRIM", "1") != "0"
_GROUP_FUSED = os.environ.get("DOCQA_GROUP_FUSED", "0") == "1"
_PREFILL_MID = os.environ.get("DOCQA_PREFILL_MID", "1") != "0"


@dataclass
class LlamaConfig:
    name: str = "llama3-8b"
    vocab_size: int = 128256
    hidden: int = 4096
    intermediate: int = 14336
    layers: int = 32
    heads: int = 32
    kv_heads: int = 8
    head_dim: int = 128
    rope_theta: float = 500000.0
    rms_eps: float = 1e-5
    max_position: int = 8192
    bos_token_id: int = 128000
    eos_token_id: int = 128009
    rope_scaling: dict | None = None
    sliding_window: int | None = None

    @staticmethod
    def preset(name: str) -> "LlamaConfig":
        if name in ("llama3-8b", "llama-3-8b", "8b"):
            return LlamaConfig()
        if name in ("llama3-70b", "llama-3-70b", "70b"):
            return LlamaConfig(name="llama3-70b", hidden=8192, intermediate=28672, layers=80,
                               heads=64, kv_heads=8)
        if name in ("mistral-7b", "mistral"):
            return LlamaConfig(name="mistral-7b", vocab_size=32768, rope_theta=1e6, max_position=32768,
                               bos_token_id=1, eos_token_id=2)
        if name == "llama3-1b-test":
            return LlamaConfig(name=name, vocab_size=32000, hidden=2048, intermediate=8192,
                               layers=4, heads=16, kv_heads=4, max_position=4096,
                               bos_token_id=1, eos_token_id=2)
        if name == "test-tp8":
            return LlamaConfig(name=name, vocab_size=4000, hidden=1024, intermediate=2048,
                               layers=2, heads=32, kv_heads=8, head_dim=128, max_position=2048,
                               bos_token_id=1, eos_token_id=2)
        if name == "tiny":
            return LlamaConfig(name="tiny", vocab_size=4096, hidden=256, intermediate=512,
                               layers=2, heads=4, kv_heads=2, head_dim=128, max_position=2048,
                               bos_token_id=1, eos_token_id=2)
        if name == "tiny-8k":
            return LlamaConfig(name="tiny-8k", vocab_size=4096, hidden=256, intermediate=512,
                               layers=2, heads=4, kv_heads=2, head_dim=128, max_position=8192,
                               bos_token_id=1, eos_token_id=2)
        raise ValueError(f"unknown llama preset {name}")

    def num_params(self) -> int:
        H, I, D = self.hidden, self.intermediate, self.head_dim
        per_layer = H * (self.heads + 2 * self.kv_heads) * D + self.heads * D * H + 3 * H * I + 2 * H
        return self.layers * per_layer + 2 * self.vocab_size * H + H


@dataclass
class AttnMeta:
    prefill: bool
    positions: torch.Tensor
    slot_mapping: torch.Tensor
    cu_seqlens: torch.Tensor | None = None
    max_len: int = 0
    block_tables: torch.Tensor | None = None
    context_lens: torch.Tensor | None = None
    max_context: int = 0
    prefix_lens: torch.Tensor | None = None
    shared_table: torch.Tensor | None = None
    shared_len: torch.Tensor | None = None
    cascade_chunks: int = 8
    seq_order: torch.Tensor | None = None
    decode_groups: torch.Tensor | None = None
    decode_defer: bool = False
    decode_inline: bool = False


class Streamed(NamedTuple):
    fmt: str
    layers: list
    lm_head: tuple


@dataclass
class StepPlan:
    proj: dict = field(default_factory=dict)
    glu: tuple = ("prefill_glu",)
    streamed: dict = field(default_factory=dict)
    nf: dict = field(default_factory=dict)
    xn: bool = False

    def splits(self, k: str) -> int:
        return self.proj[k][1] if k in self.proj else 0


class LlamaModel:
    def __init__(self, cfg: LlamaConfig, device="cuda", dtype=torch.bfloat16, seed: int = 0,
                 init: bool = True):
        self.cfg = cfg
        self.device = torch.device(device)
        self.dtype = dtype
        ps = comm.state()
        self.tp = ps.tp_size
        self.tp_rank = ps.tp_rank
        if cfg.heads % self.tp or cfg.kv_heads % self.tp or cfg.intermediate % self.tp:
            raise ValueError("heads / kv_heads / intermediate must divide the TP size")
        self.hq = cfg.heads // self.tp
        self.hkv = cfg.kv_heads // self.tp
        self.inter = cfg.intermediate // self.tp
        self.vocab_shard = (cfg.vocab_size + self.tp - 1) // self.tp
        if self.tp > 1:
            self.vocab_shard = (self.vocab_shard + 255) // 256 * 256
        self.vocab_start = self.tp_rank * self.vocab_shard
        self.vocab_valid = max(0, min(cfg.vocab_size - self.vocab_start, self.vocab_shard))
        self.scale = 1.0 / math.sqrt(cfg.head_dim)
        self.cos_sin = ops.rope_cos_sin(cfg.max_position, cfg.head_dim, cfg.rope_theta, self.device,
                                        scaling=cfg.rope_scaling)
        self.layers: list[dict] = []
        self._tick = None
        self._ntick = None
        self.streamed: Streamed | None = None
        if init:
            self._random_init(seed)

    def _random_init(self, seed: int) -> None:
        cfg, dev, dt = self.cfg, self.device, self.dtype
        g = torch.Generator(device=dev)
        std = 0.02
        out_std = std / math.sqrt(2 * cfg.layers)
        H, D, r = cfg.hidden, cfg.head_dim, self.tp_rank

        def gen(key, shape, s=std):
            g.manual_seed((seed * 1_000_003 + zlib.crc32(repr(key).encode())) & 0x7FFFFFFFFFFF)
            t = torch.empty(*shape, device=dev, dtype=dt)
            t.normal_(0.0, s, generator=g)
            return t

        def rows(key, lo, hi, width, blk, s=std):
            return torch.cat([gen(key + (b,), (blk, width), s) for b in range(lo // blk, hi // blk)])

        ib = 64 if self.inter % 64 == 0 else 8
        self.embed = gen(("embed",), (cfg.vocab_size, H))
        self.final_norm = torch.ones(H, device=dev, dtype=dt)
        vb = next(b for b in (256, 8, 1) if cfg.vocab_size % b == 0)
        self.lm_head = rows(("lm",), self.vocab_start, self.vocab_start + self.vocab_shard, H, vb)
        if self.vocab_valid < self.vocab_shard:
            self.lm_head[self.vocab_valid:] = 0
        i0, i1 = r * self.inter, (r + 1) * self.inter
        for li in range(cfg.layers):
            q = rows((li, "q"), r * self.hq * D, (r + 1) * self.hq * D, H, D)
            k = rows((li, "k"), r * self.hkv * D, (r + 1) * self.hkv * D, H, D)
            v = rows((li, "v"), r * self.hkv * D, (r + 1) * self.hkv * D, H, D)
            o = rows((li, "o"), r * self.hq * D, (r + 1) * self.hq * D, H, D, out_std).t()
            gt = rows((li, "gate"), i0, i1, H, ib)
            up = rows((li, "up"), i0, i1, H, ib)
            dn = rows((li, "down"), i0, i1, H, ib, out_std).t()
            self.layers.append({
                "in_norm": torch.ones(H, device=dev, dtype=dt),
# ... 191 lines not shown
        fam, S, r, b16 = p
        if fam.startswith("streamed_"):
            return ops.streamed_partial(self.streamed.fmt, fam[9:], a, w, S, r)
        if fam == "gemv":
            return ops.gemv_partial(a, w, S, r)
        if fam == "mgemm" and S == 1:
            return ops.mgemm_partial(a, w, 1, r).float()[None]
        if fam == "mgemm":
            return ops.mgemm_partial(a, w, S, r, bf16=b16)
        if fam == "dgemm":
            return ops.dgemm_partial(a, w, S, r)
        if fam == "pgemm":
            return ops.pgemm_partial(a, w, S)
        if fam == "linear32":
            return F.linear(a.float(), w.float())[None]
        raise ValueError(f"no kernel family {fam!r}")

    def _glu(self, plan: StepPlan, a, w):
        fam, *args = plan.glu
        if fam.startswith("streamed_"):
            return ops.streamed_glu(self.streamed.fmt, fam[9:], a, w)
        return getattr(ops, fam)(a, w, *args)

    def forward(self, input_ids: torch.Tensor, meta: AttnMeta, kv_caches: list,
                logits_index: torch.Tensor | None = None, greedy_ids: bool = False) -> torch.Tensor:
        cfg = self.cfg
        D, hq, hkv, eps = cfg.head_dim, self.hq, self.hkv, cfg.rms_eps
        h, x = ops.embed_rmsnorm(input_ids, self.embed, self.layers[0]["in_norm"], eps)
        residual = h
        nl = len(self.layers)
        decode = not meta.prefill
        kv8 = bool(kv_caches) and ops.kv_is_fp8(kv_caches[0][0])
        group_fused, cascade_rope = _GROUP_FUSED and not kv8, _CASCADE_ROPE and not kv8
        lin = ops.decode_linear if decode else ops.prefill_linear
        M = x.shape[0]
        cascade = decode and meta.shared_len is not None
        plan = self._step_plan(M, meta, x.is_cuda, kv8,
                               fused_attn=(decode and not cascade and meta.block_tables is not None
                                           and bool(kv_caches)
                                           and ops.fused_decode_ok(kv_caches[0][0], meta.block_tables)))
        sq, so, sd = plan.splits("qkv"), plan.splits("o"), plan.splits("down")
        nf, xn = plan.nf, plan.xn
        fmt = self.streamed.fmt if plan.streamed else ""
        if nf and self._ntick is None:
            self._ntick = torch.zeros(1, dtype=torch.int32, device=self.device)
        trim = (not decode and _PREFILL_TRIM and x.is_cuda and logits_index is not None and self.layers
                and meta.block_tables is not None and meta.prefix_lens is not None
                and logits_index.numel() == meta.block_tables.shape[0] and M > logits_index.numel())
        res2 = torch.empty_like(residual) if xn else None
        pd = None
        for i, L in enumerate(self.layers):
            kc, vc = kv_caches[i]
            if plan.streamed:
                L = {**L, **{k: self.streamed.layers[i][k] for k in plan.streamed}}
            if sq:
                if xn and pd is not None:
                    Sg, R = ops.gemv_plan(M, *self.layers[i]["qkv"].shape)
                    if "qkv" in plan.streamed:
                        qkv_slabs = ops.streamed_partial_xn(fmt, plan.streamed["qkv"], pd, residual, res2,
                                                            L["in_norm"], eps, L["qkv"], sq, plan.proj["qkv"][2])
                    elif Sg == sq:
                        qkv_slabs = ops.gemv_partial_xn(pd, residual, res2, L["in_norm"], eps, L["qkv"], sq, R)
                    else:
                        qkv_slabs = ops.dgemm_partial_xn(pd, residual, res2, L["in_norm"], eps, L["qkv"], sq)
                    residual, res2 = res2, residual
                else:
                    qkv_slabs = self._partial(plan.proj["qkv"], x, L["qkv"])
            if cascade:
                if (sq and meta.decode_groups is not None and meta.decode_inline and x.is_cuda
                        and group_fused and meta.slot_mapping is not None):
                    a = ops.paged_decode_grouped_fused(qkv_slabs, meta.positions, self.cos_sin, meta.slot_mapping,
                                                       kc, vc, meta.block_tables, meta.context_lens, hq,
                                                       self.scale, meta.shared_table, meta.shared_len,
                                                       meta.cascade_chunks, meta.decode_groups, self._decode_tick(M))
                elif sq:
                    qkv = ops.rope_cache_splitk(qkv_slabs, meta.positions,
                                                self.cos_sin, meta.slot_mapping, kc, vc, hq, hkv, D)
                    if meta.decode_groups is not None:
                        a = ops.paged_decode_cascade_grouped(qkv, kc, vc, meta.block_tables, meta.context_lens,
                                                             hq, self.scale, meta.shared_table, meta.shared_len,
                                                             meta.cascade_chunks, meta.decode_groups,
                                                             meta.decode_defer,
                                                             self._decode_tick(M) if x.is_cuda else None,
                                                             meta.decode_inline)
                    else:
                        a = ops.paged_decode_cascade(qkv, kc, vc, meta.block_tables, meta.context_lens, hq,
                                                     meta.max_context, self.scale, meta.shared_table,
                                                     meta.shared_len, meta.cascade_chunks, meta.seq_order)
                elif not cascade_rope:
                    qkv = lin(x, L["qkv"])
                    ops.rope_cache(qkv, meta.positions, self.cos_sin, meta.slot_mapping, kc, vc, hq, hkv, D)
                    if meta.decode_groups is not None:
                        a = ops.paged_decode_cascade_grouped(qkv, kc, vc, meta.block_tables, meta.context_lens,
                                                             hq, self.scale, meta.shared_table, meta.shared_len,
                                                             meta.cascade_chunks, meta.decode_groups,
                                                             meta.decode_defer,
                                                             self._decode_tick(M) if x.is_cuda else None,
                                                             meta.decode_inline)
                    else:
                        a = ops.paged_decode_cascade(qkv, kc, vc, meta.block_tables, meta.context_lens, hq,
                                                     meta.max_context, self.scale, meta.shared_table,
                                                     meta.shared_len, meta.cascade_chunks, meta.seq_order)
                else:
                    a = ops.paged_decode_cascade_rope(lin(x, L["qkv"]), meta.positions, self.cos_sin,
                                                      meta.slot_mapping, kc, vc, meta.block_tables,
                                                      meta.context_lens, hq, meta.max_context, self.scale,
                                                      meta.shared_table, meta.shared_len,
                                                      meta.cascade_chunks, meta.seq_order)
                qkv = None
            elif decode and sq and ops.fused_decode_ok(kc, meta.block_tables):
                a = ops.paged_decode_fused(qkv_slabs, meta.positions, self.cos_sin,
                                           meta.slot_mapping, kc, vc, meta.block_tables, meta.context_lens,
                                           hq, meta.max_context, self.scale, meta.seq_order,
                                           self._decode_tick(M) if x.is_cuda else None)
                qkv = None
            elif sq:
                qkv = ops.rope_cache_splitk(qkv_slabs, meta.positions, self.cos_sin,
                                            meta.slot_mapping, kc, vc, hq, hkv, D)
            else:
                qkv = lin(x, L["qkv"])
                ops.rope_cache(qkv, meta.positions, self.cos_sin, meta.slot_mapping, kc, vc, hq, hkv, D)
            if trim and i == nl - 1 and qkv is not None:
                ctx = meta.prefix_lens + (meta.cu_seqlens[1:] - meta.cu_seqlens[:-1])
                a = ops.paged_decode(qkv.index_select(0, logits_index).contiguous(), kc, vc, meta.block_tables,
                                     ctx, hq, meta.block_tables.shape[1] * kc.shape[2], self.scale)
                residual = residual.index_select(0, logits_index)
                logits_index = None
                qkv = None
            if qkv is None:
                pass
            elif meta.prefill and meta.prefix_lens is not None:
                a = ops.flash_prefill_paged(qkv, meta.cu_seqlens, meta.max_len, hq, hkv, D, self.scale,
                                            kc, vc, meta.block_tables, meta.prefix_lens)
            elif meta.prefill:
                a = ops.flash_prefill(qkv, meta.cu_seqlens, meta.max_len, hq, hkv, D, self.scale, True)
            else:
                a = ops.paged_decode(qkv, kc, vc, meta.block_tables, meta.context_lens, hq,
                                     meta.max_context, self.scale, meta.seq_order)
            nxt = self.layers[i + 1]["in_norm"] if i + 1 < nl else self.final_norm
            if xn:
                po = self._partial(plan.proj["o"], a, L["o"])
                if "gate_up" in plan.streamed:
                    g = ops.streamed_glu_xn(fmt, plan.streamed["gate_up"], po, residual, res2, L["post_norm"], eps,
                                            L["gate_up"])
                elif ops.gemv_glu_ok(M, *L["gate_up"].shape):
                    g = ops.gemv_glu_xn(po, residual, res2, L["post_norm"], eps, L["gate_up"])
                else:
                    g = ops.dgemm_glu_xn(po, residual, res2, L["post_norm"], eps, L["gate_up"])
                residual, res2 = res2, residual
                pd = self._partial(plan.proj["down"], g, L["down"])
                if i + 1 == nl:
                    x = ops.add_rmsnorm_splitk(pd, residual, nxt, eps)
                continue
            if "o" in nf:
                x = ops.dgemm_add_rmsnorm(a, L["o"], nf["o"], residual, L["post_norm"], eps, self._ntick)
            else:
                x = comm.tp_add_rmsnorm(self._partial(plan.proj["o"], a, L["o"]) if so else lin(a, L["o"]),
                                        residual, L["post_norm"], eps)
            g = self._glu(plan, x, L["gate_up"])
            if "down" in nf:
                x = ops.dgemm_add_rmsnorm(g, L["down"], nf["down"], residual, nxt, eps, self._ntick)
            else:
                x = comm.tp_add_rmsnorm(self._partial(plan.proj["down"], g, L["down"]) if sd else lin(g, L["down"]),
                                        residual, nxt, eps)
        if logits_index is not None:
            x = x.index_select(0, logits_index)
        if greedy_ids:
            return self.greedy_ids(x)
        return ops.lm_head_logits(x, self.lm_head)

    def forward_mixed(self, input_ids: torch.Tensor, n_dec: int, dmeta: AttnMeta, pmeta: AttnMeta,
                      kv_caches: list, logits_index: torch.Tensor, return_logits: bool = False) -> torch.Tensor:
        cfg = self.cfg
        D, hq, hkv, eps = cfg.head_dim, self.hq, self.hkv, cfg.rms_eps
        h, x = ops.embed_rmsnorm(input_ids, self.embed, self.layers[0]["in_norm"], eps)
        residual = h
        positions = torch.cat([dmeta.positions, pmeta.positions]) if n_dec else pmeta.positions
        slots = torch.cat([dmeta.slot_mapping, pmeta.slot_mapping]) if n_dec else pmeta.slot_mapping
        nl = len(self.layers)
        M = x.shape[0]
        for i, L in enumerate(self.layers):
            kc, vc = kv_caches[i]
            qkv = ops.prefill_linear(x, L["qkv"])
            ops.rope_cache(qkv, positions, self.cos_sin, slots, kc, vc, hq, hkv, D)
            parts = []
            if n_dec:
                parts.append(self._attend_decode(qkv[:n_dec], dmeta, kc, vc, n_dec))
            parts.append(ops.flash_prefill_paged(qkv[n_dec:], pmeta.cu_seqlens, pmeta.max_len, hq, hkv, D,
                                                 self.scale, kc, vc, pmeta.block_tables, pmeta.prefix_lens))
            a = torch.cat(parts) if len(parts) > 1 else parts[0]
            nxt = self.layers[i + 1]["in_norm"] if i + 1 < nl else self.final_norm
            x = comm.tp_add_rmsnorm(ops.prefill_linear(a, L["o"]), residual, L["post_norm"], eps)
            g = ops.prefill_glu(x, L["gate_up"])
            x = comm.tp_add_rmsnorm(ops.prefill_linear(g, L["down"]), residual, nxt, eps)
        assert x.shape[0] == M
        if return_logits:
            return ops.lm_head_logits(x.index_select(0, logits_index).contiguous(), self.lm_head)
        return self.greedy_ids(x.index_select(0, logits_index))

    def _attend_decode(self, qkv: torch.Tensor, meta: AttnMeta, kc, vc, M: int) -> torch.Tensor:
        hq = self.hq
        if meta.shared_len is not None:
            if meta.decode_groups is not None:
                return ops.paged_decode_cascade_grouped(qkv, kc, vc, meta.block_tables, meta.context_lens, hq,
                                                        self.scale, meta.shared_table, meta.shared_len,
                                                        meta.cascade_chunks, meta.decode_groups, meta.decode_defer,
                                                        self._decode_tick(M) if qkv.is_cuda else None,
                                                        meta.decode_inline)
            return ops.paged_decode_cascade(qkv, kc, vc, meta.block_tables, meta.context_lens, hq,
                                            meta.max_context, self.scale, meta.shared_table, meta.shared_len,
                                            meta.cascade_chunks, meta.seq_order)
        return ops.paged_decode(qkv, kc, vc, meta.block_tables, meta.context_lens, hq, meta.max_context,
                                self.scale, meta.seq_order)

    def _decode_tick(self, B: int):
        import os

        mult = max(1, int(os.environ.get("DOCQA_GROUP_CAP_MULT", "1")))
        need = max(B, 1) * mult * self.hkv
        if self._tick is None:
            self._tick = ops.decode_ticket(max(B, 4096) * mult * self.hkv, self.device)
        if self._tick.numel() < need:
            raise RuntimeError(f"decode ticket buffer holds {self._tick.numel()} words, a {B}-row bucket "
                               f"needs {need}: raise the first bucket size (buffers are never regrown)")
        return self._tick

    def greedy_ids(self, x: torch.Tensor) -> torch.Tensor:
        R = x.shape[0]
        N, K = self.lm_head.shape
        fused = ops.lm_head_argmax_ok(R, N, K) or (self.tp > 1 and 0 < R <= ops.MID_M_MAX
                                                   and ops.lm_head_argmax_shape_ok(N, K))
        if self.tp == 1:
            if fused:
                s = self.streamed
                return ops.lm_head_argmax(x, self.lm_head, self.cfg.vocab_size,
                                          streamed=(s.fmt, s.lm_head) if s is not None else None)
            return self.greedy(ops.lm_head_logits(x, self.lm_head))
        if fused and self.vocab_valid > 0:
            ids, vals = ops.lm_head_argmax(x, self.lm_head, self.vocab_valid, with_values=True)
        else:
            logits = ops.lm_head_logits(x, self.lm_head)[:, : max(1, self.vocab_valid)]
            ids = ops.argmax(logits)
            vals = logits.gather(1, ids[:, None])[:, 0].float()
        if self.vocab_valid == 0:
            vals = torch.full_like(vals, float("-inf"))
        return comm.tp_argmax(vals, ids + self.vocab_start)

    def greedy(self, logits: torch.Tensor) -> torch.Tensor:
        if self.tp == 1:
            return ops.argmax(logits)
        valid = logits[:, : max(1, self.vocab_valid)]
        idx = ops.argmax(valid)
        val = valid.gather(1, idx[:, None])[:, 0].float()
        if self.vocab_valid == 0:
            val = torch.full_like(val, float("-inf"))
        return comm.tp_argmax(val, idx + self.vocab_start)

    def full_logits(self, logits: torch.Tensor) -> torch.Tensor:
        full = comm.tp_all_gather_last(logits)
        return full[:, : self.cfg.vocab_size]
```

### docqa-ms-clinical-document-qa-assistant-llm-microservices-_amd/ops/__init__.py

```python
from __future__ import annotations

import os
import threading
from pathlib import Path
from typing import Callable, NamedTuple

import torch

from . import reference as ref

_LIB_PATH = Path(os.environ.get("DOCQA_NATIVE_LIB") or Path(__file__).resolve().parent / "_docqa_C.so")
_lock = threading.Lock()
_loaded = False
_load_error: str | None = None
_FORCE_REF = os.environ.get("DOCQA_FORCE_REFERENCE", "0") == "1"


def library_path() -> Path:
    return _LIB_PATH


def load_native(build_if_missing: bool = False) -> bool:
    global _loaded, _load_error
    if _loaded:
# ... 945 lines not shown

PENALTY_WINDOW = ref.PENALTY_WINDOW


def apply_penalties(logits, hist, hist_n, last_n, rep_pen, pres_pen, freq_pen, valid=None) -> None:
    if _gpu(logits):
        _native().apply_penalties(logits, hist, hist_n, last_n, rep_pen, pres_pen, freq_pen, valid)
        return
    ref.apply_penalties(logits, hist, hist_n, last_n, rep_pen, pres_pen, freq_pen, valid)


def penalized_argmax(logits, n_valid: int, hist, hist_n, last_n, rep_pen, pres_pen, freq_pen, valid=None):
    if _gpu(logits):
        return _native().penalized_argmax(logits, int(n_valid), hist, hist_n, last_n, rep_pen, pres_pen,
                                          freq_pen, valid)
    return ref.penalized_argmax(logits, n_valid, hist, hist_n, last_n, rep_pen, pres_pen, freq_pen, valid)


TOP_LOGPROBS_MAX = ref.TOP_LOGPROBS_MAX


def token_logprobs(logits, n_valid: int, chosen, top_n, lp=None, top_ids=None, top_lp=None):
    R, dev = logits.shape[0], logits.device
    if lp is None:
        lp = torch.zeros(R, dtype=torch.float32, device=dev)
    if top_ids is None:
        top_ids = torch.full((R, TOP_LOGPROBS_MAX), -1, dtype=torch.int32, device=dev)
    if top_lp is None:
        top_lp = torch.full((R, TOP_LOGPROBS_MAX), float("-inf"), dtype=torch.float32, device=dev)
    if _gpu(logits):
        _native().token_logprobs(logits, int(n_valid), chosen, top_n, lp, top_ids, top_lp)
    else:
        ref.token_logprobs(logits, int(n_valid), chosen, top_n, lp, top_ids, top_lp)
    return lp, top_ids, top_lp


def decode_advance_hist(nxt, out, tokens, positions, context_lens, valid, hist, hist_n) -> None:
    if _gpu(nxt):
        _native().decode_advance_hist(nxt, out, tokens, positions, context_lens, valid, hist, hist_n)
        return
    ref.decode_advance_hist(nxt, out, tokens, positions, context_lens, valid, hist, hist_n)


def paged_decode(q, k_cache, v_cache, block_tables, context_lens, Hq, max_context, scale, order=None):
    if _gpu(q):
        return _native().paged_decode(q, k_cache, v_cache, block_tables, context_lens, Hq,
                                      max_context, scale, order)
    return ref.paged_decode(q, k_cache, v_cache, block_tables, context_lens, Hq, max_context, scale)


def cascade_ok(k_cache, block_tables, Hq: int) -> bool:
    if not _gpu(k_cache):
        return Hq % k_cache.shape[1] == 0
    if kv_is_fp8(k_cache):
        return False
    return (k_cache.shape[2] == 64 and k_cache.shape[3] == 128 and Hq == 4 * k_cache.shape[1]
            and block_tables.shape[1] <= 256)


def paged_decode_cascade_rope(qkv, positions, cos_sin, slot_mapping, k_cache, v_cache, block_tables,
                              context_lens, Hq, max_context, scale, prefix_table, prefix_len,
                              nchunk: int = 8, order=None):
    if _gpu(qkv):
        return _native().paged_decode_cascade_rope(qkv, positions, cos_sin, slot_mapping, k_cache, v_cache,
                                                   block_tables, context_lens, Hq, max_context, scale,
                                                   prefix_table, prefix_len, nchunk, order)
    Hkv, D = k_cache.shape[1], k_cache.shape[3]
    ref.rope_cache(qkv, positions, cos_sin, slot_mapping, k_cache, v_cache, Hq, Hkv, D)
    return ref.paged_decode_cascade(qkv, k_cache, v_cache, block_tables, context_lens, Hq, max_context,
                                    scale, prefix_table, prefix_len, nchunk)


def paged_decode_cascade(q, k_cache, v_cache, block_tables, context_lens, Hq, max_context, scale,
                         prefix_table, prefix_len, nchunk: int = 8, order=None):
    if _gpu(q):
        return _native().paged_decode_cascade(q, k_cache, v_cache, block_tables, context_lens, Hq,
                                              max_context, scale, prefix_table, prefix_len, nchunk, order)
    return ref.paged_decode_cascade(q, k_cache, v_cache, block_tables, context_lens, Hq, max_context,
                                    scale, prefix_table, prefix_len, nchunk)


def paged_decode_cascade_grouped(q, k_cache, v_cache, block_tables, context_lens, Hq, scale,
                                 prefix_table, prefix_len, nchunk: int, groups, defer: bool = False,
                                 tick=None, inline_prefix: bool = False):
    if _gpu(q):
        if groups.dim() == 3:
            return _native().paged_decode_cascade_split(q, k_cache, v_cache, block_tables, context_lens, Hq,
                                                        scale, prefix_table, prefix_len, nchunk, groups,
                                                        defer and groups.shape[0] == 2, tick,
                                                        bool(inline_prefix) and groups.shape[0] == 2)
        return _native().paged_decode_cascade_grouped(q, k_cache, v_cache, block_tables, context_lens, Hq,
                                                      scale, prefix_table, prefix_len, nchunk, groups)
    max_context = block_tables.shape[1] * k_cache.shape[2]
    return ref.paged_decode_cascade(q, k_cache, v_cache, block_tables, context_lens, Hq, max_context,
                                    scale, prefix_table, prefix_len, nchunk)


def paged_decode_grouped_fused(P, positions, cos_sin, slot_mapping, k_cache, v_cache, block_tables, context_lens,
                               Hq, scale, prefix_table, prefix_len, nchunk: int, plan, tick=None):
    if _gpu(P):
        return _native().paged_decode_grouped_fused(P, positions, cos_sin, slot_mapping, k_cache, v_cache,
                                                    block_tables, context_lens, Hq, scale, prefix_table,
                                                    prefix_len, nchunk, plan, tick)
    Hkv, D = k_cache.shape[1], k_cache.shape[3]
    qkv = rope_cache_splitk(P, positions, cos_sin, slot_mapping, k_cache, v_cache, Hq, Hkv, D)
    return paged_decode_cascade_grouped(qkv, k_cache, v_cache, block_tables, context_lens, Hq, scale, prefix_table,
                                        prefix_len, nchunk, plan, False, tick, True)


GROUP_MAX_BLOCKS = 64


def grouped_decode_ok(k_cache, block_tables, Hq: int, max_blocks: int | None = None) -> bool:
    nb = block_tables.shape[1] if max_blocks is None else max_blocks
    if _gpu(k_cache) and kv_is_fp8(k_cache):
        return (k_cache.shape[2] == 64 and k_cache.shape[3] == 128 and Hq == 4 * k_cache.shape[1]
                and block_tables.shape[1] <= 256 and nb <= GROUP_MAX_BLOCKS)
    return cascade_ok(k_cache, block_tables, Hq) and nb <= GROUP_MAX_BLOCKS


def pack_decode_groups(tables: list[list[int]], lens: list[int], skip: int, block_size: int,
                       cap: int) -> list[list[int]]:
    n = len(tables)
    if n == 0:
        return []
    label: dict[int, int] = {}
    for t in tables:
        for b in t[skip:]:
            label.setdefault(b, len(label))
    keyed = [[label[b] for b in t[skip:]] for t in tables]
    idx = sorted(range(n), key=lambda i: keyed[i])

    def first(i):
        return tables[i][skip] if len(tables[i]) > skip else -1 - i

    clusters, cur = [], [idx[0]]
    for a, b in zip(idx, idx[1:]):
        if first(a) == first(b) and first(a) >= 0:
            cur.append(b)
        else:
            clusters.append(cur)
            cur = [b]
    clusters.append(cur)
    quads, cur = [], []
    for cl in clusters:
        while len(cl) > 4:
            quads.append(cl[:4])
            cl = cl[4:]
        if len(cur) + len(cl) > 4:
            quads.append(cur)
            cur = []
        cur = cur + cl
    if cur:
        quads.append(cur)
    if len(quads) > cap:
        quads = [idx[i:i + 4] for i in range(0, n, 4)]

    def work(qd):
        blocks = set()
        for r in qd:
            nb = (lens[r] + block_size - 1) // block_size
            blocks.update(tables[r][skip:nb])
        return len(blocks)

    quads.sort(key=work, reverse=True)
    return quads


def kv_copy_rows(pools: list, copies: list, ptrs: torch.Tensor | None = None) -> None:
    if not copies:
        return
    k0 = pools[0][0]
    if _gpu(k0):
        if ptrs is None:
            ptrs = torch.tensor([t.data_ptr() for kv in pools for t in kv], dtype=torch.int64, device=k0.device)
        tab = torch.tensor(copies, dtype=torch.int32).pin_memory().to(k0.device, non_blocking=True)
        copy = _native().kv_copy_rows8 if kv_is_fp8(k0) else _native().kv_copy_rows
        copy(ptrs, tab, k0.shape[0], k0.shape[1], k0.shape[2], k0.shape[3])
        return
    src = torch.tensor([s for s, _, m in copies for _ in range(m)], dtype=torch.long, device=k0.device)
    dst = torch.tensor([d for _, d, m in copies for _ in range(m)], dtype=torch.long, device=k0.device)
    rows = torch.tensor([i for _, _, m in copies for i in range(m)], dtype=torch.long, device=k0.device)
    for kc, vc in pools:
        if kv_is_fp8(kc):
            kc, vc = kc.view(torch.uint8), vc.view(torch.uint8)
        kc[dst, :, rows] = kc[src, :, rows]
        vc[dst, :, rows] = vc[src, :, rows]


def group_tiles_by_position(tables: list[list[int]], lens: list[int], rows: list[int], skip: int,
                            block_size: int) -> list[tuple[int, int]]:
    half = block_size // 2
    rl = [(tables[r], lens[r]) for r in rows]
# ... 154 lines not shown
```

### docqa-ms-clinical-document-qa-assistant-llm-microservices-_amd/ops/reference.py

```python
from __future__ import annotations

import math

import torch
import torch.nn.functional as F


def rmsnorm(x, w, eps):
    xf = x.float()
    inv = torch.rsqrt(xf.pow(2).mean(-1, keepdim=True) + eps)
    return (xf * inv * w.float()).to(x.dtype)


def add_rmsnorm(x, residual, w, eps):
    s = (x.float() + residual.float()).to(x.dtype)
    residual.copy_(s)
    return rmsnorm(s, w, eps)


def layernorm(x, residual, gamma, beta, eps):
    xf = x.float()
    if residual is not None:
        xf = xf + residual.float()
    return F.layer_norm(xf, (x.shape[-1],), gamma.float(), beta.float(), eps).to(x.dtype)
# ... 275 lines not shown
            s = s.masked_fill(mask, -math.inf)
        o = torch.einsum("hlm,hmd->hld", torch.softmax(s, -1), v)
        out[s0:s1] = o.transpose(0, 1).reshape(L, Hq * D).to(qkv.dtype)
    return out


def flash_prefill_paged(qkv, cu_seqlens, max_len, Hq, Hkv, D, scale, k_cache, v_cache,
                        block_tables, ctx_start):
    T = qkv.shape[0]
    x = qkv.view(T, Hq + 2 * Hkv, D)
    G = Hq // Hkv
    BS = k_cache.shape[2]
    out = torch.empty(T, Hq * D, dtype=qkv.dtype, device=qkv.device)
    cu = cu_seqlens.tolist()
    for b in range(len(cu) - 1):
        s0, s1 = cu[b], cu[b + 1]
        L = s1 - s0
        if L == 0:
            continue
        P0 = int(ctx_start[b])
        Lk = P0 + L
        nblk = (Lk + BS - 1) // BS
        blocks = block_tables[b, :nblk].long()
        k = _kv_gather(k_cache, blocks).permute(1, 0, 2, 3).reshape(Hkv, nblk * BS, D)[:, :Lk].float()
        v = _kv_gather(v_cache, blocks).permute(1, 0, 2, 3).reshape(Hkv, nblk * BS, D)[:, :Lk].float()
        k = k.repeat_interleave(G, 0)
        v = v.repeat_interleave(G, 0)
        q = x[s0:s1, :Hq].float().transpose(0, 1)
        s = torch.einsum("hld,hmd->hlm", q, k) * scale
        qpos = torch.arange(P0, Lk, device=qkv.device)[:, None]
        kpos = torch.arange(Lk, device=qkv.device)[None, :]
        s = s.masked_fill(kpos > qpos, -math.inf)
        o = torch.einsum("hlm,hmd->hld", torch.softmax(s, -1), v)
        out[s0:s1] = o.transpose(0, 1).reshape(L, Hq * D).to(qkv.dtype)
    return out


def knn(xb, xb_norms, xq, k, inner_product, id_offset):
    nq = xq.shape[0]
    N = xb.shape[0]
    D = torch.full((nq, k), -3.4028234663852886e38 if inner_product else 3.4028234663852886e38,
                   dtype=torch.float32, device=xq.device)
    I = torch.full((nq, k), -1, dtype=torch.long, device=xq.device)
    if N == 0 or nq == 0:
        return D, I
    xbf = xb.float()
    xqf = xq.float()
    ip = xqf @ xbf.T
    if inner_product:
        vals, idx = torch.topk(ip, min(k, N), dim=1, largest=True)
    else:
        norms = xb_norms.float() if xb_norms is not None else (xbf * xbf).sum(1)
        d = (xqf * xqf).sum(1, keepdim=True) + norms[None, :] - 2 * ip
        vals, idx = torch.topk(d, min(k, N), dim=1, largest=False)
    D[:, : vals.shape[1]] = vals
    I[:, : idx.shape[1]] = idx + id_offset
    return D, I


def pool_l2(h, cu_seqlens, mean, normalize):
    cu = cu_seqlens.tolist()
    out = torch.zeros(len(cu) - 1, h.shape[-1], dtype=torch.float32, device=h.device)
    for b in range(len(cu) - 1):
        s0, s1 = cu[b], cu[b + 1]
        if s1 > s0:
            out[b] = h[s0:s1].float().mean(0) if mean else h[s0].float()
    if normalize:
        out = F.normalize(out, dim=-1, eps=1e-12)
    return out


def decode_slots(block_tables, positions, valid, BS: int):
    blk = torch.gather(block_tables, 1, (positions // BS).long().clamp(max=block_tables.shape[1] - 1)[:, None])[:, 0]
    return torch.where(valid.bool(), blk * BS + positions % BS, torch.full_like(blk, -1)).int()


def decode_advance(nxt, out, tokens, positions, context_lens, valid) -> None:
    out.copy_(nxt)
    tokens.copy_(nxt.int())
    positions.add_(valid)
    context_lens.add_(valid)


PENALTY_WINDOW = 256


def penalty_neutral(last_n: int, rp: float, pp: float, fp: float) -> bool:
    return last_n == 0 or (rp == 1.0 and pp == 0.0 and fp == 0.0)


def _window_counts(hist_row, hist_n: int, last_n: int, V: int) -> dict:
    W = hist_row.numel()
    n = max(0, min(hist_n, W))
    if 0 <= last_n < n:
        n = last_n
    ring = hist_row.tolist()
    counts: dict = {}
    for j in range(hist_n - n, hist_n):
        t = ring[j % W]
        if 0 <= t < V:
            counts[t] = counts.get(t, 0) + 1
    return counts


def _penalize_row(x, counts: dict, rp, pp, fp) -> None:
    for t, c in counts.items():
        l = x[t]
        l = l * rp if bool(l <= 0) else l / rp
        x[t] = l - (torch.tensor(float(c), dtype=torch.float32) * fp + pp)


def _row_params(r, hist_n, last_n, rep_pen, pres_pen, freq_pen):
    f32 = lambda v: v[r].detach().to("cpu", torch.float32)
    return int(hist_n[r]), int(last_n[r]), f32(rep_pen), f32(pres_pen), f32(freq_pen)


def apply_penalties(logits, hist, hist_n, last_n, rep_pen, pres_pen, freq_pen, valid=None) -> None:
    assert logits.dtype == torch.float32
    V = logits.shape[1]
    for r in range(logits.shape[0]):
        hn, ln, rp, pp, fp = _row_params(r, hist_n, last_n, rep_pen, pres_pen, freq_pen)
        if (valid is not None and int(valid[r]) == 0) or penalty_neutral(ln, float(rp), float(pp), float(fp)):
            continue
        counts = _window_counts(hist[r].cpu(), hn, ln, V)
        if counts:
            idx = torch.tensor(list(counts), dtype=torch.long)
            x = logits[r, idx].cpu()
            _penalize_row(x, {i: c for i, c in enumerate(counts.values())}, rp, pp, fp)
            logits[r, idx.to(logits.device)] = x.to(logits.device)


def penalized_argmax(logits, n_valid: int, hist, hist_n, last_n, rep_pen, pres_pen, freq_pen, valid=None):
    x = logits[:, :n_valid].float().clone()
    apply_penalties(x, hist, hist_n, last_n, rep_pen, pres_pen, freq_pen, valid)
    return x.argmax(dim=-1)


TOP_LOGPROBS_MAX = 20


def token_logprobs(logits, n_valid: int, chosen, top_n, lp, top_ids, top_lp) -> None:
    x = logits[:, :n_valid].float()
    for r in range(x.shape[0]):
        tn = min(int(top_n[r]), TOP_LOGPROBS_MAX)
        if tn < 0:
            continue
        d = x[r] - x[r].max()
        rel = d - torch.log(torch.exp(d).sum())
        c = int(chosen[r])
        lp[r] = rel[c] if 0 <= c < n_valid else -math.inf
        top_ids[r] = -1
        top_lp[r] = -math.inf
        k = min(tn, n_valid)
        if k > 0:
            ids = torch.sort(x[r], descending=True, stable=True).indices[:k]
            top_ids[r, :k] = ids.to(top_ids.dtype)
            top_lp[r, :k] = rel[ids]


def decode_advance_hist(nxt, out, tokens, positions, context_lens, valid, hist, hist_n) -> None:
    W = hist.shape[1]
    rows = torch.nonzero(valid.bool())[:, 0]
    hist[rows, (hist_n[rows] % W).long()] = nxt[rows].int()
    hist_n.add_(valid)
    decode_advance(nxt, out, tokens, positions, context_lens, valid)

# ... 6 lines not shown
```

Before: 187.4 queries/s.

## Precompute per-group decode tile lists once per step and reuse across layers

Adds a decode_tile_lists kernel that builds each group's KV tile list, row lengths and header once per decode step into a persistent buffer. The grouped split-decode attention kernel gains a PRE variant that loads this record with vector loads into shared memory. This replaces the per-layer wave-0 block-table scan, prefix scan and extra synchronisation, and overlaps the q load with the record fetch. In exchange it adds one small launch per step and a buffer of cap × TILE_REC ints that is never regrown, and the path is gated by an environment flag.

```diff
diff --git a/docqa-ms-clinical-document-qa-assistant-llm-microservices-_amd/csrc/bindings.cpp b/docqa-ms-clinical-document-qa-assistant-llm-microservices-_amd/csrc/bindings.cpp
--- a/docqa-ms-clinical-document-qa-assistant-llm-microservices-_amd/csrc/bindings.cpp
+++ b/docqa-ms-clinical-document-qa-assistant-llm-microservices-_amd/csrc/bindings.cpp
@@ -685,7 +685,8 @@
                                       const at::Tensor& block_tables, const at::Tensor& context_lens,
                                       int64_t Hq, double scale, const at::Tensor& prefix_table,
                                       const at::Tensor& prefix_len, int64_t nchunk, const at::Tensor& plan,
-                                      bool defer, const c10::optional<at::Tensor>& tick, bool inline_prefix) {
+                                      bool defer, const c10::optional<at::Tensor>& tick, bool inline_prefix,
+                                      const c10::optional<at::Tensor>& tiles) {
   CHECK_GPU(q); CHECK_BF16(q);
   TORCH_CHECK(k_cache.dim() == 4, "k_cache: [num_blocks, Hkv, BS, D]");
   const bool f8 = kv_fp8(k_cache, v_cache, k_cache.size(1), k_cache.size(3));
@@ -719,6 +720,14 @@
     TORCH_CHECK(tick->numel() >= (int64_t)cap * Hkv, "split decode: tick needs cap * Hkv entries");
     tick_ptr = tick->data_ptr<int>();
   }
+  const unsigned* tiles_ptr = nullptr;
+  if (tiles && tiles->defined() && plan.size(0) == 2) {
+    CHECK_GPU((*tiles)); CHECK_I32((*tiles)); CHECK_CONTIG((*tiles));
+    TORCH_CHECK(tiles->dim() == 2 && tiles->size(0) >= cap && tiles->size(1) == docqa_decode_tile_rec(),
+                "split decode: tiles [>= cap, tile record] (decode_tile_lists)");
+    CHECK_ALIGN16((*tiles));
+    tiles_ptr = reinterpret_cast<const unsigned*>(tiles->data_ptr<int>());
+  }
   if (f8) {
     TORCH_CHECK(q.dim() == 2 && q.size(1) >= Hq * D && q.stride(0) % 8 == 0, "split decode (fp8 cache): q rows");
     CHECK_ALIGN16(q);
@@ -726,7 +735,7 @@
                                             block_tables.data_ptr<int>(), block_tables.size(1),
                                             context_lens.data_ptr<int>(), out.data_ptr(), Hq * D, B, Hq, Hkv, BS,
                                             (float)scale, pp, pp + 8 * cap, cap, ws_acc.data_ptr<float>(),
-                                            ws_ml.data_ptr<float>(), stream(), tick_ptr),
+                                            ws_ml.data_ptr<float>(), stream(), tick_ptr, tiles_ptr),
              "paged_decode_cascade_split (fp8 cache)");
     return out;
   }
@@ -748,9 +757,38 @@
                                             prefix_len.data_ptr<int>(), (int)nchunk, pacc.data_ptr<float>(),
                                             pml.data_ptr<float>(), pp, pp + 8 * cap, cap, ws_acc.data_ptr<float>(),
                                             ws_ml.data_ptr<float>(), defer ? 1 : 0, stream(), tick_ptr,
-                                            inline_prefix ? 1 : 0),
+                                            inline_prefix ? 1 : 0, nullptr, 0, nullptr, nullptr, nullptr, tiles_ptr),
            "paged_decode_cascade_split");
   return out;
+}
+
+int64_t decode_tile_rec() { return docqa_decode_tile_rec(); }
+
+void decode_tile_lists(const at::Tensor& plan, const at::Tensor& block_tables, const at::Tensor& context_lens,
+                       const c10::optional<at::Tensor>& prefix_len, at::Tensor out) {
+  CHECK_GPU(plan); CHECK_I32(plan); CHECK_CONTIG(plan);
+  CHECK_GPU(block_tables); CHECK_I32(block_tables); CHECK_CONTIG(block_tables);
+  CHECK_GPU(context_lens); CHECK_I32(context_lens); CHECK_CONTIG(context_lens);
+  CHECK_GPU(out); CHECK_I32(out); CHECK_CONTIG(out);
+  TORCH_CHECK(plan.dim() == 3 && plan.size(0) >= 2 && plan.size(2) == 8 && plan.size(1) >= 1,
+              "decode_tile_lists: split plan [2, cap, 8]");
+  const int cap = plan.size(1), B = context_lens.numel();
+  TORCH_CHECK(block_tables.dim() == 2 && block_tables.size(0) >= B && block_tables.size(1) >= 1 &&
+              block_tables.size(1) <= 256, "decode_tile_lists: block tables [>= B, 1..256]");
+  TORCH_CHECK(out.dim() == 2 && out.size(0) >= cap && out.size(1) == docqa_decode_tile_rec(),
+              "decode_tile_lists: out [>= cap, tile record]");
+  CHECK_ALIGN16(out);
+  const int* plen = nullptr;
+  if (prefix_len && prefix_len->defined()) {
+    CHECK_GPU((*prefix_len)); CHECK_I32((*prefix_len));
+    TORCH_CHECK(prefix_len->numel() == 1, "decode_tile_lists: one prefix length");
+    plen = prefix_len->data_ptr<int>();
+  }
+  c10::DeviceGuard g(plan.device());
+  CHECK_RC(docqa_decode_tile_lists(plan.data_ptr<int>(), cap, block_tables.data_ptr<int>(), block_tables.size(1),
+                                   context_lens.data_ptr<int>(), B, plen,
+                                   reinterpret_cast<unsigned*>(out.data_ptr<int>()), stream()),
+           "decode_tile_lists");
 }
 
 at::Tensor paged_decode_cascade_rope(at::Tensor qkv, const at::Tensor& positions, const at::Tensor& cos_sin,
@@ -1825,7 +1863,11 @@
   m.def("kv_copy_rows8(Tensor caches, Tensor tab, int num_blocks, int Hkv, int BS, int D) -> ()");
   m.def("paged_decode_cascade_split(Tensor q, Tensor k_cache, Tensor v_cache, Tensor block_tables, "
         "Tensor context_lens, int Hq, float scale, Tensor prefix_table, Tensor prefix_len, int nchunk, "
-        "Tensor plan, bool defer=False, Tensor(t!)? tick=None, bool inline_prefix=False) -> Tensor");
+        "Tensor plan, bool defer=False, Tensor(t!)? tick=None, bool inline_prefix=False, Tensor? tiles=None) "
+        "-> Tensor");
+  m.def("decode_tile_rec() -> int", &decode_tile_rec);
+  m.def("decode_tile_lists(Tensor plan, Tensor block_tables, Tensor context_lens, Tensor? prefix_len, "
+        "Tensor(a!) out) -> ()");
   m.def("paged_decode_grouped_fused(Tensor P, Tensor positions, Tensor cos_sin, Tensor slot_mapping, "
         "Tensor(a!) k_cache, Tensor(b!) v_cache, Tensor block_tables, Tensor context_lens, int Hq, float scale, "
         "Tensor prefix_table, Tensor prefix_len, int nchunk, Tensor plan, Tensor(t!)? tick=None) -> Tensor");
@@ -1919,6 +1961,7 @@
   m.impl("paged_decode_cascade_rope", &paged_decode_cascade_rope);
   m.impl("paged_decode_cascade_grouped", &paged_decode_cascade_grouped);
   m.impl("paged_decode_cascade_split", &paged_decode_cascade_split);
+  m.impl("decode_tile_lists", &decode_tile_lists);
   m.impl("paged_decode_grouped_fused", &paged_decode_grouped_fused);
   m.impl("kv_copy_rows", &kv_copy_rows);
   m.impl("kv_copy_rows8", &kv_copy_rows8);
diff --git a/docqa-ms-clinical-document-qa-assistant-llm-microservices-_amd/csrc/include/docqa_kernels.h b/docqa-ms-clinical-document-qa-assistant-llm-microservices-_amd/csrc/include/docqa_kernels.h
--- a/docqa-ms-clinical-document-qa-assistant-llm-microservices-_amd/csrc/include/docqa_kernels.h
+++ b/docqa-ms-clinical-document-qa-assistant-llm-microservices-_amd/csrc/include/docqa_kernels.h
@@ -36,7 +36,7 @@
                                    const int* block_tables, int maxb, const int* context_lens, void* out,
                                    int out_stride, int B, int Hq, int Hkv, int BS, float scale, const int* items,
                                    const int* merges, int cap, float* ws_acc, float* ws_ml, hipStream_t s,
-                                   int* tick);
+                                   int* tick, const unsigned* tiles = nullptr);
 
 int docqa_silu_mul(const void* gu, void* out, int T, int I, int interleaved, hipStream_t s);
 int docqa_silu_mul_splitk16(const void* P, void* out, int S, int T, int I, hipStream_t s);
@@ -104,7 +104,11 @@
                                      float* ws_acc, float* ws_ml, int defer,
                                      hipStream_t s, int* tick = nullptr, int inline_prefix = 0,
                                      const float* fP = nullptr, int fS = 0, const int* positions = nullptr,
-                                     const float* cos_sin = nullptr, const int* slot_mapping = nullptr);
+                                     const float* cos_sin = nullptr, const int* slot_mapping = nullptr,
+                                     const unsigned* tiles = nullptr);
+int docqa_decode_tile_rec();
+int docqa_decode_tile_lists(const int* items, int cap, const int* block_tables, int maxb, const int* context_lens,
+                            int B, const int* plen, unsigned* out, hipStream_t s);
 int docqa_paged_decode_cascade_persist(const void* q, int q_stride, void* k_cache, void* v_cache,
                                        const int* block_tables, int maxb, const int* context_lens,
                                        void* out, int out_stride, int B, int Hq, int Hkv, int BS,
diff --git a/docqa-ms-clinical-document-qa-assistant-llm-microservices-_amd/csrc/kernels/attn_decode.hip b/docqa-ms-clinical-document-qa-assistant-llm-microservices-_amd/csrc/kernels/attn_decode.hip
--- a/docqa-ms-clinical-document-qa-assistant-llm-microservices-_amd/csrc/kernels/attn_decode.hip
+++ b/docqa-ms-clinical-document-qa-assistant-llm-microservices-_amd/csrc/kernels/attn_decode.hip
@@ -1237,20 +1237,106 @@
   return __uint_as_float(b.x) + __uint_as_float(b.y);
 }
 
-template <int WAVES, int NSRW>
+__device__ __forceinline__ int group_wave_tile_list(const int (&rows)[4], const int (&Ls)[4], int P, int lo, int hi,
+                                                    const int* __restrict__ block_tables, int maxb, int lane,
+                                                    unsigned* tl) {
+  constexpr int R = 4, TQ = 16;
+  const int pos = max(P >> 6, lo) + lane;
+  int ids[R], nq[R], mk[R];
+#pragma unroll
+  for (int r = 0; r < R; ++r) ids[r] = rows[r] >= 0 && pos < hi ? block_tables[(size_t)rows[r] * maxb + pos] : -1;
+  bool alive[R];
+#pragma unroll
+  for (int r = 0; r < R; ++r) {
+    alive[r] = pos < hi && 64 * pos < Ls[r];
+    ids[r] = alive[r] ? ids[r] : -1;
+  }
+  int cnt = 0;
+#pragma unroll
+  for (int r = 0; r < R; ++r) {
+    bool first = alive[r];
+#pragma unroll
+    for (int r2 = 0; r2 < r; ++r2) first = first && !(alive[r2] && ids[r2] == ids[r]);
+    int mask = 0, need = 0;
+    if (first) {
+#pragma unroll
+      for (int r2 = 0; r2 < R; ++r2)
+        if (alive[r2] && ids[r2] == ids[r]) {
+          mask |= 1 << r2;
+          need = max(need, min(4, (Ls[r2] - 64 * pos + TQ - 1) / TQ));
+        }
+    }
+    nq[r] = need;
+    mk[r] = mask;
+    cnt += need;
+  }
+  int off = cnt;
+#pragma unroll
+  for (int o = 1; o < 64; o <<= 1) {
+    const int v = __shfl_up(off, o, 64);
+    if (lane >= o) off += v;
+  }
+  const int total = __shfl(off, 63, 64);
+  off -= cnt;
+#pragma unroll
+  for (int r = 0; r < R; ++r)
+    for (int h = 0; h < nq[r]; ++h) tl[off++] = ((unsigned)ids[r] << 12) | (pos << 6) | (h << 4) | mk[r];
+  return total;
+}
+
+constexpr int kTileHdr = 16;
+constexpr int kTileRec = kTileHdr + kGroupMaxPos * 16;
+
+__global__ __launch_bounds__(64) void decode_tile_lists_kernel(const int* __restrict__ groups,
+                                                               const int* __restrict__ block_tables, int maxb,
+                                                               const int* __restrict__ context_lens, int B,
+                                                               const int* __restrict__ plen,
+                                                               unsigned* __restrict__ out) {
+  constexpr int R = 4;
+  const int lane = threadIdx.x;
+  const int* gp = groups + 8 * blockIdx.x;
+  unsigned* rec = out + (size_t)blockIdx.x * kTileRec;
+  const int P = plen ? *plen : 0;
+  int rows[R], Ls[R];
+#pragma unroll
+  for (int r = 0; r < R; ++r) {
+    const int row = gp[r];
+    rows[r] = row >= 0 && row < B ? row : -1;
+    Ls[r] = rows[r] >= 0 ? context_lens[rows[r]] : 0;
+  }
+  const bool used = rows[0] >= 0 || rows[1] >= 0 || rows[2] >= 0 || rows[3] >= 0;
+  const int lo = gp[4], hi = min(gp[5], maxb), part = gp[6];
+  const int nt = used ? group_wave_tile_list(rows, Ls, P, lo, hi, block_tables, maxb, lane, rec + kTileHdr) : 0;
+  if (lane < kTileHdr) {
+    int w = 0;
+#pragma unroll
+    for (int r = 0; r < R; ++r) {
+      if (lane == r) w = rows[r];
+      if (lane == R + r) w = Ls[r];
+    }
+    if (lane == 8) w = nt;
+    if (lane == 9) w = part;
+    if (lane == 10) w = P;
+    rec[lane] = (unsigned)w;
+  }
+  for (int i = nt + lane; i < kGroupMaxPos * 16; i += 64) rec[kTileHdr + i] = 0u;
+}
+
+template <int WAVES, int NSRW, bool PRE = false>
 __global__ __launch_bounds__(64 * WAVES) void paged_decode_group_wave_kernel(
     const uint16_t* __restrict__ q, int q_stride, const uint16_t* __restrict__ k_cache,
     const uint16_t* __restrict__ v_cache, const int* __restrict__ block_tables, int maxb,
     const int* __restrict__ context_lens, int B, int Hkv, float scale,
     uint16_t* __restrict__ out, int out_stride, const int* __restrict__ groups, CascadeIn ci,
-    float* __restrict__ ws_acc, float* __restrict__ ws_ml, const int* __restrict__ merges, int* __restrict__ tick) {
+    float* __restrict__ ws_acc, float* __restrict__ ws_ml, const int* __restrict__ merges, int* __restrict__ tick,
+    const unsigned* __restrict__ tiles = nullptr) {
   constexpr int G = 4, R = 4, D = 128, TQ = 16, MAXT = kGroupMaxPos * 16;
   constexpr int TILE = TQ * D;
   constexpr int WSLOT = 2 * TILE;
   constexpr int NDT = 8 / WAVES;
   static_assert(WAVES * NSRW * WSLOT * 2 >= WAVES * 8 * 64 * 16 + WAVES * 16 * 2 * 4, "ring reused by the merge");
   __shared__ __attribute__((aligned(16))) uint16_t ring[WAVES * NSRW * WSLOT];
-  __shared__ unsigned s_tl[MAXT];
+  __shared__ __attribute__((aligned(16))) unsigned s_tl[MAXT];
   __shared__ int s_nt;
 
   const int kvh = blockIdx.x, grp = blockIdx.y;
@@ -1260,73 +1346,64 @@
   long long* trace = g_group_trace;
   long long tr0 = 0, tr1 = 0, tr2 = 0, tr3 = 0;
   if (trace && tid == 0) tr0 = wall_clock64();
-  const int P = ci.plen ? *ci.plen : 0;
   const int* gp = groups + 8 * grp;
-  int rows[R], Ls[R];
-#pragma unroll
-  for (int r = 0; r < R; ++r) {
-    const int row = gp[r];
-    rows[r] = row >= 0 && row < B ? row : -1;
-    Ls[r] = rows[r] >= 0 ? context_lens[rows[r]] : 0;
-  }
-  if (rows[0] < 0 && rows[1] < 0 && rows[2] < 0 && rows[3] < 0) return;
-  const int lo = gp[4], hi = min(gp[5], maxb), part = gp[6];
-
-  if (wave == 0) {
-    const int pos = max(P >> 6, lo) + lane;
-    int ids[R], nq[R], mk[R];
-#pragma unroll
-    for (int r = 0; r < R; ++r) ids[r] = rows[r] >= 0 && pos < hi ? block_tables[(size_t)rows[r] * maxb + pos] : -1;
-    bool alive[R];
+  int P, part, nt, rows[R], Ls[R];
+  bf16x8 qf[4];
+  if constexpr (PRE) {
+    const unsigned* rec = tiles + (size_t)grp * kTileRec;
+    constexpr int NV = MAXT / 4 / (64 * WAVES);
+    uint4 ev[NV];
+#pragma unroll
+    for (int k = 0; k < NV; ++k)
+      ev[k] = *reinterpret_cast<const uint4*>(rec + kTileHdr + 4 * (tid + k * 64 * WAVES));
 #pragma unroll
     for (int r = 0; r < R; ++r) {
-      alive[r] = pos < hi && 64 * pos < Ls[r];
-      ids[r] = alive[r] ? ids[r] : -1;
-    }
-    int cnt = 0;
+      rows[r] = (int)rec[r];
+      Ls[r] = (int)rec[R + r];
+    }
+    nt = (int)rec[8];
+    part = (int)rec[9];
+    P = (int)rec[10];
+    {
+      const int crow = rows[hl >> 2];
+      const uint16_t* qp = q + (size_t)max(crow, 0) * q_stride + (size_t)(kvh * G + (hl & 3)) * D + lg * 8;
+#pragma unroll
+      for (int ks = 0; ks < 4; ++ks) {
+        const uint4 v = crow >= 0 ? *reinterpret_cast<const uint4*>(qp + ks * 32) : make_uint4(0, 0, 0, 0);
+        qf[ks] = __builtin_bit_cast(bf16x8, v);
+      }
+    }
+#pragma unroll
+    for (int k = 0; k < NV; ++k) *reinterpret_cast<uint4*>(s_tl + 4 * (tid + k * 64 * WAVES)) = ev[k];
+    if (rows[0] < 0 && rows[1] < 0 && rows[2] < 0 && rows[3] < 0) return;
+    __syncthreads();
+  } else {
+    P = ci.plen ? *ci.plen : 0;
 #pragma unroll
     for (int r = 0; r < R; ++r) {
-      bool first = alive[r];
-#pragma unroll
-      for (int r2 = 0; r2 < r; ++r2) first = first && !(alive[r2] && ids[r2] == ids[r]);
-      int mask = 0, need = 0;
-      if (first) {
-#pragma unroll
-        for (int r2 = 0; r2 < R; ++r2)
-          if (alive[r2] && ids[r2] == ids[r]) {
-            mask |= 1 << r2;
-            need = max(need, min(4, (Ls[r2] - 64 * pos + TQ - 1) / TQ));
-          }
-      }
-      nq[r] = need;
-      mk[r] = mask;
-      cnt += need;
-    }
-    int off = cnt;
-#pragma unroll
-    for (int o = 1; o < 64; o <<= 1) {
-      const int v = __shfl_up(off, o, 64);
-      if (lane >= o) off += v;
-    }
-    const int total = __shfl(off, 63, 64);
-    off -= cnt;
-#pragma unroll
-    for (int r = 0; r < R; ++r)
-      for (int h = 0; h < nq[r]; ++h) s_tl[off++] = ((unsigned)ids[r] << 12) | (pos << 6) | (h << 4) | mk[r];
-    if (lane == 0) s_nt = total;
+      const int row = gp[r];
+      rows[r] = row >= 0 && row < B ? row : -1;
+      Ls[r] = rows[r] >= 0 ? context_lens[rows[r]] : 0;
+    }
+    if (rows[0] < 0 && rows[1] < 0 && rows[2] < 0 && rows[3] < 0) return;
+    const int lo = gp[4], hi = min(gp[5], maxb);
+    part = gp[6];
+    if (wave == 0) {
+      const int total = group_wave_tile_list(rows, Ls, P, lo, hi, block_tables, maxb, lane, s_tl);
+      if (lane == 0) s_nt = total;
+    }
   }
   const int crow = rows[hl >> 2], cL = Ls[hl >> 2], cbit = 1 << (hl >> 2);
-  bf16x8 qf[4];
-  {
+  if constexpr (!PRE) {
     const uint16_t* qp = q + (size_t)max(crow, 0) * q_stride + (size_t)(kvh * G + (hl & 3)) * D + lg * 8;
 #pragma unroll
     for (int ks = 0; ks < 4; ++ks) {
       const uint4 v = crow >= 0 ? *reinterpret_cast<const uint4*>(qp + ks * 32) : make_uint4(0, 0, 0, 0);
       qf[ks] = __builtin_bit_cast(bf16x8, v);
     }
-  }
-  __syncthreads();
-  const int nt = s_nt;
+    __syncthreads();
+    nt = s_nt;
+  }
   if (trace && tid == 0) tr1 = wall_clock64();
 
   const float qs = scale * kLog2e;
@@ -1453,93 +1530,80 @@
   return __builtin_bit_cast(i16x4, u);
 }
 
-template <int NSRW>
+template <int NSRW, bool PRE = false>
 __global__ __launch_bounds__(256) void paged_decode_group_wave8_kernel(
     const uint16_t* __restrict__ q, int q_stride, const uint8_t* __restrict__ k_cache,
     const uint8_t* __restrict__ v_cache, const int* __restrict__ block_tables, int maxb,
     const int* __restrict__ context_lens, int B, int Hkv, float scale,
     uint16_t* __restrict__ out, int out_stride, const int* __restrict__ groups, CascadeIn ci,
-    float* __restrict__ ws_acc, float* __restrict__ ws_ml, const int* __restrict__ merges, int* __restrict__ tick) {
+    float* __restrict__ ws_acc, float* __restrict__ ws_ml, const int* __restrict__ merges, int* __restrict__ tick,
+    const unsigned* __restrict__ tiles = nullptr) {
   constexpr int WAVES = 4, G = 4, R = 4, D = 128, TQ = 16, MAXT = kGroupMaxPos * 16;
   constexpr int TILE = TQ * D;
   constexpr int WSLOT = 2 * TILE;
   constexpr int NDT = 8 / WAVES;
   static_assert(WAVES * NSRW * WSLOT >= WAVES * 8 * 64 * 16 + WAVES * 16 * 2 * 4, "ring reused by the merge");
   __shared__ __attribute__((aligned(16))) uint8_t ring[WAVES * NSRW * WSLOT];
-  __shared__ unsigned s_tl[MAXT];
+  __shared__ __attribute__((aligned(16))) unsigned s_tl[MAXT];
   __shared__ int s_nt;
 
   const int kvh = blockIdx.x, grp = blockIdx.y;
   const int tid = threadIdx.x, lane = tid & 63;
   const int wave = __builtin_amdgcn_readfirstlane(tid >> 6);
   const int hl = lane & 15, lg = lane >> 4;
-  const int P = ci.plen ? *ci.plen : 0;
   const int* gp = groups + 8 * grp;
-  int rows[R], Ls[R];
-#pragma unroll
-  for (int r = 0; r < R; ++r) {
-    const int row = gp[r];
-    rows[r] = row >= 0 && row < B ? row : -1;
-    Ls[r] = rows[r] >= 0 ? context_lens[rows[r]] : 0;
-  }
-  if (rows[0] < 0 && rows[1] < 0 && rows[2] < 0 && rows[3] < 0) return;
-  const int lo = gp[4], hi = min(gp[5], maxb), part = gp[6];
-
-  if (wave == 0) {
-    const int pos = max(P >> 6, lo) + lane;
-    int ids[R], nq[R], mk[R];
-#pragma unroll
-    for (int r = 0; r < R; ++r) ids[r] = rows[r] >= 0 && pos < hi ? block_tables[(size_t)rows[r] * maxb + pos] : -1;
-    bool alive[R];
+  int P, part, nt, rows[R], Ls[R];
+  bf16x8 qf[4];
+  if constexpr (PRE) {
+    const unsigned* rec = tiles + (size_t)grp * kTileRec;
+    const uint4 ev = *reinterpret_cast<const uint4*>(rec + kTileHdr + 4 * tid);
 #pragma unroll
     for (int r = 0; r < R; ++r) {
-      alive[r] = pos < hi && 64 * pos < Ls[r];
-      ids[r] = alive[r] ? ids[r] : -1;
-    }
-    int cnt = 0;
+      rows[r] = (int)rec[r];
+      Ls[r] = (int)rec[R + r];
+    }
+    nt = (int)rec[8];
+    part = (int)rec[9];
+    P = (int)rec[10];
+    {
+      const int crow = rows[hl >> 2];
+      const uint16_t* qp = q + (size_t)max(crow, 0) * q_stride + (size_t)(kvh * G + (hl & 3)) * D + lg * 8;
+#pragma unroll
+      for (int ks = 0; ks < 4; ++ks) {
+        const uint4 v = crow >= 0 ? *reinterpret_cast<const uint4*>(qp + ks * 32) : make_uint4(0, 0, 0, 0);
+        qf[ks] = __builtin_bit_cast(bf16x8, v);
+      }
+    }
+    *reinterpret_cast<uint4*>(s_tl + 4 * tid) = ev;
+    if (rows[0] < 0 && rows[1] < 0 && rows[2] < 0 && rows[3] < 0) return;
+    __syncthreads();
+  } else {
+    P = ci.plen ? *ci.plen : 0;
 #pragma unroll
     for (int r = 0; r < R; ++r) {
-      bool first = alive[r];
-#pragma unroll
-      for (int r2 = 0; r2 < r; ++r2) first = first && !(alive[r2] && ids[r2] == ids[r]);
-      int mask = 0, need = 0;
-      if (first) {
-#pragma unroll
-        for (int r2 = 0; r2 < R; ++r2)
-          if (alive[r2] && ids[r2] == ids[r]) {
-            mask |= 1 << r2;
-            need = max(need, min(4, (Ls[r2] - 64 * pos + TQ - 1) / TQ));
-          }
-      }
-      nq[r] = need;
-      mk[r] = mask;
-      cnt += need;
-    }
-    int off = cnt;
-#pragma unroll
-    for (int o = 1; o < 64; o <<= 1) {
-      const int v = __shfl_up(off, o, 64);
-      if (lane >= o) off += v;
-    }
-    const int total = __shfl(off, 63, 64);
-    off -= cnt;
-#pragma unroll
-    for (int r = 0; r < R; ++r)
-      for (int h = 0; h < nq[r]; ++h) s_tl[off++] = ((unsigned)ids[r] << 12) | (pos << 6) | (h << 4) | mk[r];
-    if (lane == 0) s_nt = total;
+      const int row = gp[r];
+      rows[r] = row >= 0 && row < B ? row : -1;
+      Ls[r] = rows[r] >= 0 ? context_lens[rows[r]] : 0;
+    }
+    if (rows[0] < 0 && rows[1] < 0 && rows[2] < 0 && rows[3] < 0) return;
+    const int lo = gp[4], hi = min(gp[5], maxb);
+    part = gp[6];
+    if (wave == 0) {
+      const int total = group_wave_tile_list(rows, Ls, P, lo, hi, block_tables, maxb, lane, s_tl);
+      if (lane == 0) s_nt = total;
+    }
   }
   const int crow = rows[hl >> 2], cL = Ls[hl >> 2], cbit = 1 << (hl >> 2);
-  bf16x8 qf[4];
-  {
+  if constexpr (!PRE) {
     const uint16_t* qp = q + (size_t)max(crow, 0) * q_stride + (size_t)(kvh * G + (hl & 3)) * D + lg * 8;
 #pragma unroll
     for (int ks = 0; ks < 4; ++ks) {
       const uint4 v = crow >= 0 ? *reinterpret_cast<const uint4*>(qp + ks * 32) : make_uint4(0, 0, 0, 0);
       qf[ks] = __builtin_bit_cast(bf16x8, v);
     }
-  }
-  __syncthreads();
-  const int nt = s_nt;
+    __syncthreads();
+    nt = s_nt;
+  }
 
   const float qs = scale * kLog2e;
   const uint32_t wbase = lds_u32(ring) + (uint32_t)(wave * NSRW * WSLOT);
@@ -2130,7 +2194,7 @@
                                      float* pacc, float* pml, const int* items, const int* merges, int cap,
                                      float* ws_acc, float* ws_ml, int defer, hipStream_t s, int* tick,
                                      int inline_prefix, const float* fP, int fS, const int* positions,
-                                     const float* cos_sin, const int* slot_mapping) {
+                                     const float* cos_sin, const int* slot_mapping, const unsigned* tiles) {
   if (B == 0) return 0;
   if (BS != 64 || maxb > kGroupMaxTable || Hq != 4 * Hkv || nchunk < 1 || nchunk > kCascadeMaxChunks || cap < 1)
     return -1;
@@ -2159,9 +2223,14 @@
     if (tk) return 0;
   } else if (group_wave_on()) {
 #define DOCQA_WAVE_LAUNCH(W_, N_)                                                                                 \
-  paged_decode_group_wave_kernel<W_, N_><<<dim3(Hkv, cap), 64 * W_, 0, s>>>(                                     \
-      (const uint16_t*)q, q_stride, (const uint16_t*)k_cache, (const uint16_t*)v_cache, block_tables, maxb,       \
-      context_lens, B, Hkv, scale, (uint16_t*)out, out_stride, items, ci, ws_acc, ws_ml, merges, tk)
+  if (tiles)                                                                                                      \
+    paged_decode_group_wave_kernel<W_, N_, true><<<dim3(Hkv, cap), 64 * W_, 0, s>>>(                             \
+        (const uint16_t*)q, q_stride, (const uint16_t*)k_cache, (const uint16_t*)v_cache, block_tables, maxb,     \
+        context_lens, B, Hkv, scale, (uint16_t*)out, out_stride, items, ci, ws_acc, ws_ml, merges, tk, tiles);    \
+  else                                                                                                            \
+    paged_decode_group_wave_kernel<W_, N_><<<dim3(Hkv, cap), 64 * W_, 0, s>>>(                                   \
+        (const uint16_t*)q, q_stride, (const uint16_t*)k_cache, (const uint16_t*)v_cache, block_tables, maxb,     \
+        context_lens, B, Hkv, scale, (uint16_t*)out, out_stride, items, ci, ws_acc, ws_ml, merges, tk)
     switch (g_group_wave) {
       case 2: DOCQA_WAVE_LAUNCH(2, 3); break;
       case 3: DOCQA_WAVE_LAUNCH(2, 4); break;
@@ -2190,13 +2259,18 @@
                                    const int* block_tables, int maxb, const int* context_lens, void* out,
                                    int out_stride, int B, int Hq, int Hkv, int BS, float scale, const int* items,
                                    const int* merges, int cap, float* ws_acc, float* ws_ml, hipStream_t s,
-                                   int* tick) {
+                                   int* tick, const unsigned* tiles) {
   if (B == 0) return 0;
   if (BS != 64 || maxb > kGroupMaxTable || Hq != 4 * Hkv || cap < 1) return -1;
   const CascadeIn ci{nullptr, nullptr, nullptr, 1, nullptr};
-  paged_decode_group_wave8_kernel<4><<<dim3(Hkv, cap), 256, 0, s>>>(
-      (const uint16_t*)q, q_stride, (const uint8_t*)k_cache, (const uint8_t*)v_cache, block_tables, maxb,
-      context_lens, B, Hkv, scale, (uint16_t*)out, out_stride, items, ci, ws_acc, ws_ml, merges, tick);
+  if (tiles)
+    paged_decode_group_wave8_kernel<4, true><<<dim3(Hkv, cap), 256, 0, s>>>(
+        (const uint16_t*)q, q_stride, (const uint8_t*)k_cache, (const uint8_t*)v_cache, block_tables, maxb,
+        context_lens, B, Hkv, scale, (uint16_t*)out, out_stride, items, ci, ws_acc, ws_ml, merges, tick, tiles);
+  else
+    paged_decode_group_wave8_kernel<4><<<dim3(Hkv, cap), 256, 0, s>>>(
+        (const uint16_t*)q, q_stride, (const uint8_t*)k_cache, (const uint8_t*)v_cache, block_tables, maxb,
+        context_lens, B, Hkv, scale, (uint16_t*)out, out_stride, items, ci, ws_acc, ws_ml, merges, tick);
   DOCQA_CHECK_LAUNCH();
   if (tick) return 0;
   group_split_merge_kernel<<<dim3(Hkv, (cap + 1) / 2), 256, 0, s>>>(merges, ws_acc, ws_ml, context_lens, B, Hkv,
@@ -2232,6 +2306,16 @@
 }
 
 int docqa_group_persist_bins(int cap, int Hkv) { return group_persist_bins(cap, Hkv); }
+
+int docqa_decode_tile_rec() { return kTileRec; }
+
+int docqa_decode_tile_lists(const int* items, int cap, const int* block_tables, int maxb, const int* context_lens,
+                            int B, const int* plen, unsigned* out, hipStream_t s) {
+  if (cap < 1 || maxb < 1 || maxb > kGroupMaxTable) return -1;
+  decode_tile_lists_kernel<<<cap, 64, 0, s>>>(items, block_tables, maxb, context_lens, B, plen, out);
+  DOCQA_CHECK_LAUNCH();
+  return 0;
+}
 
 int docqa_set_decode_trace(long long* buf) {
   return hipMemcpyToSymbol(HIP_SYMBOL(g_group_trace), &buf, sizeof(buf)) == hipSuccess ? 0 : -1;
diff --git a/docqa-ms-clinical-document-qa-assistant-llm-microservices-_amd/engine/llm_engine.py b/docqa-ms-clinical-document-qa-assistant-llm-microservices-_amd/engine/llm_engine.py
--- a/docqa-ms-clinical-document-qa-assistant-llm-microservices-_amd/engine/llm_engine.py
+++ b/docqa-ms-clinical-document-qa-assistant-llm-microservices-_amd/engine/llm_engine.py
@@ -159,6 +159,10 @@
 
 def _group_wave_on() -> bool:
     return os.environ.get("DOCQA_GROUP_WAVE", "1") != "0"
+
+
+def _group_tile_lists_on() -> bool:
+    return _group_wave_on() and os.environ.get("DOCQA_GROUP_TILE_LISTS", "1") == "1"
 
 
 def _defer_groups_on() -> bool:
@@ -315,6 +319,7 @@
         self.tail = TailCache(self.kv.allocator, block_size, cap) if self._use_pc and cap > 0 else None
         self._graphs: dict[tuple, _DecodeGraph] = {}
         self._pool = None
+        self._tile_buf = None
         self.stats = GenStats()
 
     @staticmethod
@@ -428,7 +433,24 @@
                                       and not _defer_groups_on())
             if self.kv_fp8 and self.device.type == "cuda" and not meta.decode_inline:
                 meta.shared_table = meta.shared_len = meta.decode_groups = None
+            if (meta.decode_groups is not None and g.groups.dim() == 3 and g.groups.shape[0] == 2
+                    and self.device.type == "cuda" and _group_tile_lists_on()
+                    and not (meta.decode_inline and not self.kv_fp8
+                             and os.environ.get("DOCQA_GROUP_FUSED", "0") == "1")):
+                meta.decode_tiles = ops.decode_tile_lists(g.groups, g.block_tables, g.context_lens,
+                                                          None if meta.decode_inline else g.shared_len,
+                                                          out=self._decode_tile_buf(g.groups.shape[1]))
         return meta
+
+    def _decode_tile_buf(self, cap: int) -> torch.Tensor:
+        if self._tile_buf is None:
+            mult = max(1, int(os.environ.get("DOCQA_GROUP_CAP_MULT", "1")))
+            self._tile_buf = torch.zeros(max(self.max_batch * mult, cap), ops.TILE_REC, dtype=torch.int32,
+                                         device=self.device)
+        if self._tile_buf.shape[0] < cap:
+            raise RuntimeError(f"decode tile-list buffer holds {self._tile_buf.shape[0]} records, a plan of {cap} "
+                               "rows needs more: raise max_batch (buffers are never regrown)")
+        return self._tile_buf
 
     def _select(self, logits, g: _DecodeGraph, full=None):
         from .. import ops
diff --git a/docqa-ms-clinical-document-qa-assistant-llm-microservices-_amd/models/llama.py b/docqa-ms-clinical-document-qa-assistant-llm-microservices-_amd/models/llama.py
--- a/docqa-ms-clinical-document-qa-assistant-llm-microservices-_amd/models/llama.py
+++ b/docqa-ms-clinical-document-qa-assistant-llm-microservices-_amd/models/llama.py
@@ -88,6 +88,7 @@
     decode_groups: torch.Tensor | None = None
     decode_defer: bool = False
     decode_inline: bool = False
+    decode_tiles: torch.Tensor | None = None
 
 
 class Streamed(NamedTuple):
@@ -445,7 +446,7 @@
                                                              meta.cascade_chunks, meta.decode_groups,
                                                              meta.decode_defer,
                                                              self._decode_tick(M) if x.is_cuda else None,
-                                                             meta.decode_inline)
+                                                             meta.decode_inline, meta.decode_tiles)
                     else:
                         a = ops.paged_decode_cascade(qkv, kc, vc, meta.block_tables, meta.context_lens, hq,
                                                      meta.max_context, self.scale, meta.shared_table,
@@ -459,7 +460,7 @@
                                                              meta.cascade_chunks, meta.decode_groups,
                                                              meta.decode_defer,
                                                              self._decode_tick(M) if x.is_cuda else None,
-                                                             meta.decode_inline)
+                                                             meta.decode_inline, meta.decode_tiles)
                     else:
                         a = ops.paged_decode_cascade(qkv, kc, vc, meta.block_tables, meta.context_lens, hq,
                                                      meta.max_context, self.scale, meta.shared_table,
@@ -569,7 +570,7 @@
                                                         self.scale, meta.shared_table, meta.shared_len,
                                                         meta.cascade_chunks, meta.decode_groups, meta.decode_defer,
                                                         self._decode_tick(M) if qkv.is_cuda else None,
-                                                        meta.decode_inline)
+                                                        meta.decode_inline, meta.decode_tiles)
             return ops.paged_decode_cascade(qkv, kc, vc, meta.block_tables, meta.context_lens, hq,
                                             meta.max_context, self.scale, meta.shared_table, meta.shared_len,
                                             meta.cascade_chunks, meta.seq_order)
diff --git a/docqa-ms-clinical-document-qa-assistant-llm-microservices-_amd/ops/__init__.py b/docqa-ms-clinical-document-qa-assistant-llm-microservices-_amd/ops/__init__.py
--- a/docqa-ms-clinical-document-qa-assistant-llm-microservices-_amd/ops/__init__.py
+++ b/docqa-ms-clinical-document-qa-assistant-llm-microservices-_amd/ops/__init__.py
@@ -1051,13 +1051,17 @@
 
 def paged_decode_cascade_grouped(q, k_cache, v_cache, block_tables, context_lens, Hq, scale,
                                  prefix_table, prefix_len, nchunk: int, groups, defer: bool = False,
-                                 tick=None, inline_prefix: bool = False):
+                                 tick=None, inline_prefix: bool = False, tiles=None):
     if _gpu(q):
         if groups.dim() == 3:
+            inline = bool(inline_prefix) and groups.shape[0] == 2
+            if tiles is not None:
+                return _native().paged_decode_cascade_split(q, k_cache, v_cache, block_tables, context_lens, Hq,
+                                                            scale, prefix_table, prefix_len, nchunk, groups,
+                                                            defer and groups.shape[0] == 2, tick, inline, tiles)
             return _native().paged_decode_cascade_split(q, k_cache, v_cache, block_tables, context_lens, Hq,
                                                         scale, prefix_table, prefix_len, nchunk, groups,
-                                                        defer and groups.shape[0] == 2, tick,
-                                                        bool(inline_prefix) and groups.shape[0] == 2)
+                                                        defer and groups.shape[0] == 2, tick, inline)
         return _native().paged_decode_cascade_grouped(q, k_cache, v_cache, block_tables, context_lens, Hq,
                                                       scale, prefix_table, prefix_len, nchunk, groups)
     max_context = block_tables.shape[1] * k_cache.shape[2]
@@ -1078,6 +1082,18 @@
 
 
 GROUP_MAX_BLOCKS = 64
+TILE_HDR, TILE_REC = ref.TILE_HDR, ref.TILE_REC
+
+
+def decode_tile_lists(plan, block_tables, context_lens, prefix_len=None, out=None):
+    cap = plan.shape[1]
+    if out is None:
+        out = torch.empty(cap, TILE_REC, dtype=torch.int32, device=plan.device)
+    if _gpu(plan):
+        _native().decode_tile_lists(plan, block_tables, context_lens, prefix_len, out)
+    else:
+        out[:cap] = ref.decode_tile_lists(plan, block_tables, context_lens, prefix_len)
+    return out
 
 
 def grouped_decode_ok(k_cache, block_tables, Hq: int, max_blocks: int | None = None) -> bool:
diff --git a/docqa-ms-clinical-document-qa-assistant-llm-microservices-_amd/ops/reference.py b/docqa-ms-clinical-document-qa-assistant-llm-microservices-_amd/ops/reference.py
--- a/docqa-ms-clinical-document-qa-assistant-llm-microservices-_amd/ops/reference.py
+++ b/docqa-ms-clinical-document-qa-assistant-llm-microservices-_amd/ops/reference.py
@@ -381,6 +381,42 @@
     context_lens.add_(valid)
 
 
+TILE_HDR = 16
+TILE_REC = TILE_HDR + 64 * 16
+
+
+def decode_tile_lists(plan, block_tables, context_lens, prefix_len=None):
+    items = plan[0].tolist()
+    bt, cl = block_tables.tolist(), context_lens.tolist()
+    B, maxb = len(cl), block_tables.shape[1]
+    P = int(prefix_len.reshape(-1)[0]) if prefix_len is not None else 0
+    out = torch.zeros(len(items), TILE_REC, dtype=torch.int64)
+    for i, it in enumerate(items):
+        rows = [r if 0 <= r < B else -1 for r in it[:4]]
+        Ls = [cl[r] if r >= 0 else 0 for r in rows]
+        ent = []
+        if any(r >= 0 for r in rows):
+            first, hi = max(P >> 6, it[4]), min(it[5], maxb)
+            for pos in range(first, min(hi, first + 64)):
+                alive = [r >= 0 and 64 * pos < L for r, L in zip(rows, Ls)]
+                seen = []
+                for s in range(4):
+                    if not alive[s] or bt[rows[s]][pos] in seen:
+                        continue
+                    b = bt[rows[s]][pos]
+                    seen.append(b)
+                    same = [t for t in range(4) if alive[t] and bt[rows[t]][pos] == b]
+                    mask = sum(1 << t for t in same)
+                    need = max(min(4, (Ls[t] - 64 * pos + 15) // 16) for t in same)
+                    ent += [((b << 12) | (pos << 6) | (h << 4) | mask) & 0xFFFFFFFF for h in range(need)]
+        out[i, :4] = torch.tensor(rows)
+        out[i, 4:8] = torch.tensor(Ls)
+        out[i, 8], out[i, 9], out[i, 10] = len(ent), it[6], P
+        if ent:
+            out[i, TILE_HDR:TILE_HDR + len(ent)] = torch.tensor(ent, dtype=torch.int64)
+    return ((out + 2 ** 31) % 2 ** 32 - 2 ** 31).to(torch.int32)
+
+
 PENALTY_WINDOW = 256
 
 
```

After: 184.6 queries/s. 1.5% lower.
